# jhollowed/PyTEMDiags

Measured on AMD Instinct MI355X. Metric: grid-points/sec through full TEM pipeline (ncol*nlev*nt), higher is better.
Workload: dtype f64; 1 GPU; ne120 (777602 cols) x 72 lev x 30 snapshots per GPU, L=50, 1-degree zonal grid (M=180), ten GM16 Table-A1 outputs; ncol=777602, nlev=72, nt=30, sweeps=latitude-class, single sweep, mirror_paired_sweeps=True

## Files before the change

### include/temx.h

```cpp
#ifndef TEMX_H
#define TEMX_H

#include <stdint.h>

#ifdef __cplusplus
extern "C" {
#endif

typedef struct temx_plan temx_plan;

enum { TEMX_F64 = 0, TEMX_F32 = 1 };

enum {
  TEMX_OK = 0,
  TEMX_EINVAL = -1,
  TEMX_EHIP = -2,
  TEMX_ENOMEM = -3,
  TEMX_ERANK = -4,
  TEMX_ESTATE = -5,
  TEMX_EUNSUPPORTED = -6,
  TEMX_EINTERNAL = -7
};

enum {
  TEMX_DEFER_FINALIZE = 1,
  TEMX_NO_SYMMETRY = 2,
  TEMX_NO_CLASSES = 4,
  TEMX_NO_QR = 8,
  TEMX_LAT_TOL_F32 = 16
};

enum {
  TEMX_OPT_FORM = 1,
  TEMX_OPT_OS_MAP = 2,
  TEMX_OPT_OP_MAP = 3,
  TEMX_OPT_OS_SUBSAMPLE = 4,
  TEMX_OPT_TRACER_ONE_PASS = 5,
  TEMX_OPT_SINGLE_SWEEP_MIN_GROUPS = 6,
  TEMX_OPT_OS_CONTRACT = 7,
  TEMX_OPT_MISSING = 8,
  TEMX_OPT_MIN_COVERAGE = 9,
  TEMX_OPT_MISSING_WEIGHT = 10,
  TEMX_OPT_LAT_BINS = 12,
  TEMX_OPT_BIN_DEGREE = 13,
  TEMX_OPT_OS_SYNC = 11
};
enum {
  TEMX_FORM_AUTO = -1,
  TEMX_FORM_TWO_PASS = 0,
  TEMX_FORM_CLASS_SUMS = 1,
  TEMX_FORM_SINGLE_SWEEP = 2,
  TEMX_FORM_NO_SINGLE_SWEEP = 3,
  TEMX_FORM_MASKED = 4,
  TEMX_FORM_BINNED = 5
};

enum {
  TEMX_MAT_Y0 = 0,
  TEMX_MAT_Y0P = 1,
  TEMX_MAT_GRAM = 2,
  TEMX_MAT_GINV = 3,
  TEMX_MAT_Y0INV = 4,
  TEMX_MAT_GRAM2 = 5,
  TEMX_MAT_GX = 6,
  TEMX_MAT_GSUB = 7,
  TEMX_MAT_COVERAGE = 8
};

enum {
  TEMX_R_VTEM = 0, TEMX_R_OMEGATEM, TEMX_R_WTEM, TEMX_R_PSITEM, TEMX_R_EPFY, TEMX_R_EPFZ,
  TEMX_R_EPDIV, TEMX_R_UTENDEPFD, TEMX_R_UTENDVTEM, TEMX_R_UTENDWTEM, TEMX_NRESULTS
};

enum {
  TEMX_Z_UB = 0, TEMX_Z_VB, TEMX_Z_THETAB, TEMX_Z_WAPB, TEMX_Z_UPVPB, TEMX_Z_UPWAPPB,
  TEMX_Z_VPTPB, TEMX_Z_DUB_DP, TEMX_Z_DTHETAB_DP, TEMX_Z_UBCOSLAT, TEMX_Z_DUBCOSLAT_DLAT,
  TEMX_Z_PSI, TEMX_Z_PSICOSLAT, TEMX_Z_DPSICOSLAT_DLAT, TEMX_Z_DPSI_DP, TEMX_Z_INT_VBDP,
  TEMX_NZONAL
};

enum {
  TEMX_E_UP = 0, TEMX_E_VP, TEMX_E_THETAP, TEMX_E_WAPP, TEMX_E_UPVP, TEMX_E_UPWAPP, TEMX_E_VPTP,
  TEMX_NEDDY
};

int temx_version(void);
const char* temx_last_error(void);
int temx_device_count(void);

int temx_plan_create(temx_plan** out, int device, int64_t ncol, int L, int M,
                     const double* lat_deg_host, const double* lat_out_deg_host, int flags);

int temx_plan_finalize(temx_plan* plan, const double* G_host );

int temx_plan_refine(temx_plan* plan, const double* G2_host );

int temx_plan_set_weights(temx_plan* plan, const double* weights_host );

void temx_plan_destroy(temx_plan* plan);

int temx_plan_is_paired(const temx_plan* plan);
int temx_plan_sweep_mode(const temx_plan* plan);
int temx_plan_one_pass(const temx_plan* plan);
int temx_plan_single_sweep(const temx_plan* plan);

int temx_get_matrix(temx_plan* plan, int which, double* dst, void* stream);

int temx_plan_configure(temx_plan* plan, int option, int value);
int temx_plan_option(const temx_plan* plan, int option);

int temx_plan_set_os_matrices(temx_plan* plan, const double* Gx_host , const double* Gsub_host );


int temx_project(temx_plan* plan, const void* A, int dtype, int64_t D, double* B, void* stream);

int temx_zonal_mean(temx_plan* plan, const void* A, int dtype, int64_t D, double* out,
                    int native, void* stream);

int temx_zonal_mean_from_sums(temx_plan* plan, const double* B, int64_t D, double* out,
                              int native, void* stream);

int temx_plan_set_tem(temx_plan* plan, int nlev, int64_t nt, const double* p_pa_host, double p0);

int temx_tem_stage1(temx_plan* plan, const void* ua, const void* va, const void* ta,
                    const void* wap, int dtype, double* B4, void* stream);

int temx_tem_stage2(temx_plan* plan, const void* ua, const void* va, const void* ta,
                    const void* wap, int dtype, const double* B4, double* B3, void* stream);
// ... 76 lines not shown
```

### pytemdiags_amd/_lib.py

```python
from __future__ import annotations

import ctypes as C
import os

_HERE = os.path.dirname(os.path.abspath(__file__))
LIB_PATH = os.environ.get("TEMX_LIB") or os.path.join(_HERE, "libtemx.so")

ABI_VERSION = 402
F64, F32 = 0, 1
DEFER_FINALIZE = 1
NO_SYMMETRY = 2
NO_CLASSES = 4
NO_QR = 8
LAT_TOL_F32 = 16
MAT_Y0, MAT_Y0P, MAT_GRAM, MAT_GINV, MAT_Y0INV, MAT_GRAM2, MAT_GX, MAT_GSUB = 0, 1, 2, 3, 4, 5, 6, 7
MAT_COVERAGE = 8
OPT_FORM, OPT_OS_MAP, OPT_OP_MAP, OPT_OS_SUBSAMPLE, OPT_TRACER_ONE_PASS, OPT_SINGLE_SWEEP_MIN_GROUPS, OPT_OS_CONTRACT = 1, 2, 3, 4, 5, 6, 7
OPT_MISSING, OPT_MIN_COVERAGE, OPT_MISSING_WEIGHT = 8, 9, 10
OPT_OS_SYNC = 11
OPT_LAT_BINS, OPT_BIN_DEGREE = 12, 13
LAT_BINS_ALLOWED = (128, 256, 512, 1024, 2048)
LAT_BINS_DEFAULT = 512
MISSING_MODES = {"raise": 0, "mask": 1}
FORM_AUTO, FORM_TWO_PASS, FORM_CLASS_SUMS, FORM_SINGLE_SWEEP, FORM_NO_SINGLE_SWEEP = -1, 0, 1, 2, 3
FORM_MASKED = 4
FORM_BINNED = 5
FORM_NAMES = {FORM_TWO_PASS: "two-pass", FORM_CLASS_SUMS: "class-sums", FORM_SINGLE_SWEEP: "single-sweep",
              FORM_MASKED: "masked", FORM_BINNED: "binned"}
FORMS = {"auto": FORM_AUTO, "two-pass": FORM_TWO_PASS, "class-sums": FORM_CLASS_SUMS,
         "single-sweep": FORM_SINGLE_SWEEP, "no-single-sweep": FORM_NO_SINGLE_SWEEP}

RESULT_NAMES = ("vtem", "omegatem", "wtem", "psitem", "epfy", "epfz", "epdiv",
                "utendepfd", "utendvtem", "utendwtem")
ZONAL_NAMES = ("ub", "vb", "thetab", "wapb", "upvpb", "upwappb", "vptpb", "dub_dp", "dthetab_dp",
               "ubcoslat", "dubcoslat_dlat", "psi", "psicoslat", "dpsicoslat_dlat", "dpsi_dp",
               "int_vbdp")
EDDY_NAMES = ("up", "vp", "thetap", "wapp", "upvp", "upwapp", "vptp")
TRACER_RESULT_NAMES = ("etfy", "etfz", "etdiv", "qtendetfd", "qtendvtem", "qtendwtem")
TRACER_ZONAL_NAMES = ("qb", "qpvpb", "qpwappb", "dqb_dp", "qbcoslat", "dqbcoslat_dlat")
TRACER_EDDY_NAMES = ("qp", "qpvp", "qpwapp")

ERRORS = {0: "TEMX_OK", -1: "TEMX_EINVAL", -2: "TEMX_EHIP", -3: "TEMX_ENOMEM", -4: "TEMX_ERANK",
          -5: "TEMX_ESTATE", -6: "TEMX_EUNSUPPORTED", -7: "TEMX_EINTERNAL"}

_vp, _i, _i64, _dp, _u64 = C.c_void_p, C.c_int, C.c_int64, C.POINTER(C.c_double), C.c_uint64
SIGNATURES = [
    ("temx_version", _i, []),
    ("temx_last_error", C.c_char_p, []),
    ("temx_device_count", _i, []),
    ("temx_plan_create", _i, [C.POINTER(_vp), _i, _i64, _i, _i, _dp, _dp, _i]),
    ("temx_plan_finalize", _i, [_vp, _dp]),
    ("temx_plan_refine", _i, [_vp, _dp]),
    ("temx_plan_set_weights", _i, [_vp, _dp]),
    ("temx_plan_destroy", None, [_vp]),
    ("temx_plan_is_paired", _i, [_vp]),
    ("temx_plan_sweep_mode", _i, [_vp]),
    ("temx_plan_one_pass", _i, [_vp]),
    ("temx_plan_single_sweep", _i, [_vp]),
    ("temx_get_matrix", _i, [_vp, _i, _vp, _vp]),
    ("temx_plan_configure", _i, [_vp, _i, _i]),
    ("temx_plan_option", _i, [_vp, _i]),
    ("temx_plan_set_os_matrices", _i, [_vp, _dp, _dp]),
    ("temx_project", _i, [_vp, _vp, _i, _i64, _vp, _vp]),
    ("temx_zonal_mean", _i, [_vp, _vp, _i, _i64, _vp, _i, _vp]),
    ("temx_zonal_mean_from_sums", _i, [_vp, _vp, _i64, _vp, _i, _vp]),
    ("temx_plan_set_tem", _i, [_vp, _i, _i64, _dp, C.c_double]),
    ("temx_tem_stage1", _i, [_vp, _vp, _vp, _vp, _vp, _i, _vp, _vp]),
    ("temx_tem_stage2", _i, [_vp, _vp, _vp, _vp, _vp, _i, _vp, _vp, _vp]),
    ("temx_tem_stage2_from_sums", _i, [_vp, _vp, _vp, _vp]),
    ("temx_tem_stage3", _i, [_vp, _vp, _vp, _vp, _vp]),
    ("temx_tem_run", _i, [_vp, _vp, _vp, _vp, _vp, _i, _vp, _vp, _vp]),
    ("temx_tem_os_prepass", _i, [_vp, _vp, _vp, _vp, _vp, _i, _vp, _vp]),
    ("temx_tem_os_sweep", _i, [_vp, _vp, _vp, _vp, _vp, _i, _vp, _i, _vp, _vp]),
    ("temx_tem_os_tail", _i, [_vp, _vp, _i64, _i64, _vp, _vp, _vp]),
    ("temx_tracers_os_prepass", _i, [_vp, _i, C.POINTER(_vp), _vp, _vp, _i, _vp, _vp]),
    ("temx_tracers_os_sweep", _i, [_vp, _i, C.POINTER(_vp), _vp, _vp, _i, _vp, _i, _vp, _vp]),
    ("temx_tracers_os_tail", _i, [_vp, _i, _vp, C.POINTER(_vp), C.POINTER(_vp), _vp]),
    ("temx_tracers_run", _i, [_vp, _i, C.POINTER(_vp), _vp, _vp, _i, C.POINTER(_vp), C.POINTER(_vp), _vp]),
    ("temx_tem_tail_from_sums", _i, [_vp, _vp, _vp, _i64, _i64, _vp, _vp, _vp]),
    ("temx_time_slices", _i, [_vp, _vp, _i64, _i, _vp, _vp]),
    ("temx_tem_eddy", _i, [_vp, _vp, _vp, _vp, _vp, _i, C.POINTER(_vp), _vp]),
    ("temx_tem_eddy_rows", _i, [_vp, _vp, _vp, _vp, _vp, _i, _i64, _i64, C.POINTER(_vp), _vp]),
    ("temx_tracer_stage1", _i, [_vp, _vp, _i, _vp, _vp]),
    ("temx_tracer_stage2", _i, [_vp, _vp, _vp, _vp, _i, _vp, _vp, _vp]),
    ("temx_tracer_stage3", _i, [_vp, _vp, _vp, _vp, _vp]),
    ("temx_tracer_stage1_sums", _i, [_vp, _vp, _vp, _vp, _i, _vp, _vp]),
    ("temx_tracer_stage2_from_sums", _i, [_vp, _vp, _vp, _vp]),
    ("temx_tracer_run", _i, [_vp, _vp, _vp, _vp, _i, _vp, _vp, _vp]),
    ("temx_tem_tracer_stage1", _i, [_vp, _vp, _vp, _vp, _vp, _vp, _i, _vp, _vp, _vp]),
    ("temx_tem_tracer_run", _i, [_vp, _vp, _vp, _vp, _vp, _vp, _i, _vp, _vp, _vp, _vp, _vp]),
    ("temx_tracer_eddy", _i, [_vp, _vp, _vp, _vp, _i, C.POINTER(_vp), _vp]),
    ("temx_status", _i, [_vp, C.POINTER(_i), _vp]),
    ("temx_synth_fields", _i, [_i, _i64, _i, _i64, _i64, _vp, _vp, _vp, _i, _u64, _vp, _vp, _vp, _vp, _vp]),
    ("temx_mfma_f64_peak", _i, [_i, _i, _dp]),
    ("temx_kernel_timing", _i, [_vp, _i]),
    ("temx_kernel_timing_read", _i, [_vp, _i, _dp, C.POINTER(_i)]),
    ("temx_selftest_exception", _i, [_i]),
]


class TemxError(RuntimeError):
    def __init__(self, code, msg):
        super().__init__("%s (%d): %s" % (ERRORS.get(code, "TEMX_E?"), code, msg))
# ... 63 lines not shown
```

### pytemdiags_amd/csrc/kernels.hpp

```cpp
#pragma once
#include <hip/hip_runtime.h>
#include <stdint.h>

#include <type_traits>

#define TEMX_MFMA4(a, b, c) __builtin_amdgcn_mfma_f64_4x4x4f64((a), (b), (c), 0, 0, 0)

namespace temx {

template <int NF>
struct FieldPtrs {
  const void* p[NF];
};

struct EddyOut {
  double* p[7];
};

template <int KMAX>
__device__ __forceinline__ void basis_row(double xv, int K, const double* __restrict__ norm,
                                          const double* __restrict__ T, double* q) {
  double pm1 = 1.0, pc = xv;
  for (int l = 0; l < K; ++l) {
    double P;
// ... 163 lines not shown
          load_x(c0 + 1, std::integral_constant<int, (PD > 1 ? 1 : 0)>{}, ti, std::false_type{});
      }
      if (PD > 2 && c0 + 2 < c1) {
#pragma unroll
        for (int ti = 0; ti < 4; ++ti)
          load_x(c0 + 2, std::integral_constant<int, (PD > 2 ? 2 : 0)>{}, ti, std::false_type{});
      }
    }
  }
  const int cfast = (c1 < nfull ? c1 : nfull) - (2 * PD - 1);
  int chunk = c0;
  for (; chunk < cfast; chunk += PD) do_group(chunk, std::true_type{});
  for (; chunk < c1; chunk += PD) do_group(chunk, std::false_type{});

  if (dvalid) {
#pragma unroll
    for (int f = 0; f < NFW; ++f)
#pragma unroll
      for (int t = 0; t < TB; ++t) {
        const int l = t * 4 + g;
        if (l < K) partial[(((int64_t)split * NF + f0 + f) * K + l) * D + d] = acc[f][t];
      }
  }
}

struct SliceMap {
  int64_t D = 0;
  int nt = 1, W = 1;
  int64_t chunk = 0;
  int64_t row0 = 0;
};
__device__ __forceinline__ int64_t slice_index(const SliceMap& m, int64_t idx) {
  if (m.D == 0) return idx;
  const int64_t row = idx / m.D, d = idx - row * m.D;
  const int lev = (int)(d / m.nt), t = (int)(d - (int64_t)lev * m.nt);
  const int base = m.nt / m.W, extra = m.nt - base * m.W, tb = extra * (base + 1);
  int w, tl, ntw;
  if (t < tb) { w = t / (base + 1); tl = t - w * (base + 1); ntw = base + 1; }
  else { const int u = t - tb; w = extra + u / base; tl = u - (w - extra) * base; ntw = base; }
  const int nlev = (int)(m.D / m.nt);
  return (int64_t)w * m.chunk + ((m.row0 + row) * nlev + lev) * ntw + tl;
}

__global__ void __launch_bounds__(256)
reduce_partials_kernel(const double* __restrict__ partial, int nsplit, int64_t stride, int64_t n,
                       const double* __restrict__ addend, double* __restrict__ B, int* __restrict__ flag,
                       SliceMap map) {
  __shared__ double sh[16][17];
  const int e = threadIdx.x & 15, sl = threadIdx.x >> 4;
  const int64_t idx = (int64_t)blockIdx.x * 16 + e;
  double s = 0.0;
  if (idx < n)
    for (int sp = sl; sp < nsplit; sp += 16) s += partial[(int64_t)sp * stride + idx];
  sh[sl][e] = s;
  __syncthreads();
  if (sl == 0 && idx < n) {
    double t = 0.0;
#pragma unroll
    for (int j = 0; j < 16; ++j) t += sh[j][e];
    if (addend != nullptr) t += addend[idx];
    B[slice_index(map, idx)] = t;
    if (!(fabs(t) <= 1.79769313486231570815e308)) atomicOr(flag, 1);
  }
}

template <int NS>
__global__ void __launch_bounds__(256)
reduce_partials_flat_kernel(const double* __restrict__ partial, int nsplit, int64_t stride, int64_t n,
                            const double* __restrict__ addend, double* __restrict__ B, int* __restrict__ flag,
                            SliceMap map) {
  const int64_t idx = (int64_t)blockIdx.x * 256 + threadIdx.x;
  if (idx >= n) return;
  double v[NS];
#pragma unroll
  for (int sp = 0; sp < NS; ++sp) v[sp] = partial[(int64_t)(sp < nsplit ? sp : 0) * stride + idx];
  double t = 0.0;
#pragma unroll
  for (int sp = 0; sp < NS; ++sp) t += sp < nsplit ? v[sp] : 0.0;
  if (addend != nullptr) t += addend[idx];
  B[slice_index(map, idx)] = t;
  if (!(fabs(t) <= 1.79769313486231570815e308)) atomicOr(flag, 1);
}

__global__ void __launch_bounds__(256)
reduce_rows_kernel(const double* __restrict__ partial, int nsplit, int64_t stride, int nf, int rows_in, int rows,
                   int64_t D, double* __restrict__ out, int* __restrict__ flag) {
  const int64_t idx = (int64_t)blockIdx.x * 256 + threadIdx.x;
  const int64_t per = (int64_t)rows * D;
  if (idx >= per * nf) return;
  const int64_t f = idx / per, rem = idx - f * per;
  const double* src = partial + f * rows_in * D + rem;
  double t = 0.0;
  for (int sp = 0; sp < nsplit; ++sp) t += src[(int64_t)sp * stride];
  out[idx] = t;
  if (!(fabs(t) <= 1.79769313486231570815e308)) atomicOr(flag, 1);
}
__global__ void __launch_bounds__(256)
reduce_rows_wide_kernel(const double* __restrict__ partial, int nsplit, int64_t stride, int nf, int rows_in, int rows,
                        int64_t D, double* __restrict__ out, int* __restrict__ flag) {
  __shared__ double sh[16][17];
  const int e = threadIdx.x & 15, sl = threadIdx.x >> 4;
  const int64_t idx = (int64_t)blockIdx.x * 16 + e;
  const int64_t per = (int64_t)rows * D;
  const bool ok = idx < per * nf;
  double s = 0.0;
  if (ok) {
    const int64_t f = idx / per, rem = idx - f * per;
    const double* src = partial + f * rows_in * D + rem;
    for (int sp = sl; sp < nsplit; sp += 16) s += src[(int64_t)sp * stride];
  }
  sh[sl][e] = s;
  __syncthreads();
  if (sl == 0 && ok) {
    double t = 0.0;
#pragma unroll
    for (int j = 0; j < 16; ++j) t += sh[j][e];
    out[idx] = t;
    if (!(fabs(t) <= 1.79769313486231570815e308)) atomicOr(flag, 1);
  }
}

__global__ void __launch_bounds__(1024)
solve_kernel(const double* __restrict__ B, int K, int K4, int M, int64_t D,
             const double* __restrict__ Ginv, const double* __restrict__ Y0p,
             double* __restrict__ C, double* __restrict__ Xb) {
  extern __shared__ double slds[];
  double* sb = slds;
  double* scf = slds + (size_t)K4 * 17;
  const int f = blockIdx.y;
  const int64_t d0 = (int64_t)blockIdx.x * 16;
  const int tid = threadIdx.x;
  const int mper = (M + gridDim.z - 1) / gridDim.z;
  const int m0 = blockIdx.z * mper;
  const int m1 = m0 + mper < M ? m0 + mper : M;
  for (int idx = tid; idx < K * 16; idx += 1024) {
    const int k = idx >> 4, dd = idx & 15;
    const int64_t d = d0 + dd;
    sb[k * 17 + dd] = d < D ? B[((int64_t)f * K + k) * D + d] : 0.0;
  }
  __syncthreads();
  for (int idx = tid; idx < K4 * 16; idx += 1024) {
    const int k = idx >> 4, dd = idx & 15;
    const int64_t d = d0 + dd;
    double v = 0.0;
    if (k < K) {
      const double* gr = Ginv + (int64_t)k * K;
      double v0 = 0.0, v1 = 0.0, v2 = 0.0, v3 = 0.0;
      int kk = 0;
      for (; kk + 4 <= K; kk += 4) {
        v0 += gr[kk] * sb[kk * 17 + dd];
        v1 += gr[kk + 1] * sb[(kk + 1) * 17 + dd];
        v2 += gr[kk + 2] * sb[(kk + 2) * 17 + dd];
        v3 += gr[kk + 3] * sb[(kk + 3) * 17 + dd];
      }
      for (; kk < K; ++kk) v0 += gr[kk] * sb[kk * 17 + dd];
      v = (v0 + v1) + (v2 + v3);
    }
    scf[k * 17 + dd] = v;
    if (C != nullptr && blockIdx.z == 0 && d < D) C[((int64_t)f * K4 + k) * D + d] = v;
  }
  __syncthreads();
  if (Xb != nullptr) {
    for (int idx = tid; idx < (m1 - m0) * 16; idx += 1024) {
      const int m = m0 + (idx >> 4), dd = idx & 15;
      const int64_t d = d0 + dd;
      if (d >= D) continue;
      const double* yr = Y0p + (int64_t)m * K;
      double v0 = 0.0, v1 = 0.0, v2 = 0.0, v3 = 0.0;
      int kk = 0;
      for (; kk + 4 <= K; kk += 4) {
        v0 += yr[kk] * scf[kk * 17 + dd];
        v1 += yr[kk + 1] * scf[(kk + 1) * 17 + dd];
        v2 += yr[kk + 2] * scf[(kk + 2) * 17 + dd];
        v3 += yr[kk + 3] * scf[(kk + 3) * 17 + dd];
      }
      for (; kk < K; ++kk) v0 += yr[kk] * scf[kk * 17 + dd];
      Xb[((int64_t)f * M + m) * D + d] = (v0 + v1) + (v2 + v3);
    }
  }
}

constexpr int SOLVE_MB = 16;

template <int TB>
__global__ void __launch_bounds__(256)
solve_mfma_kernel(const double* __restrict__ B, int K, int M, int64_t D, const double* __restrict__ gblk,
                  const double* __restrict__ ypblk, double* __restrict__ C, double* __restrict__ Xb,
                  int mbs ) {
  extern __shared__ double slds[];
  double* sg = slds;
  double* sy = slds + TB * TB * 16;
  const int f = blockIdx.y;
  const int tid = threadIdx.x, lane = tid & 63, wave = tid >> 6;
  const int g = lane >> 4, c = lane & 15;
  const int64_t d = ((int64_t)blockIdx.x * 4 + wave) * 16 + c;
  const bool dvalid = d < D;
  const int64_t dcl = dvalid ? d : D - 1;
  const int mb0 = blockIdx.z * mbs;
  const int nmb_all = (M + 3) >> 2;
  const int nmb = Xb != nullptr ? (nmb_all - mb0 < mbs ? nmb_all - mb0 : mbs) : 0;

  double breg[TB];
#pragma unroll
  for (int t = 0; t < TB; ++t) {
    const int row = 4 * t + g;
    const int rc = row < K ? row : K - 1;
    const double v = B[((int64_t)f * K + rc) * D + dcl];
    breg[t] = row < K ? v : 0.0;
  }
  {
    constexpr int JG = (TB * TB * 16 + 255) / 256, JY = (SOLVE_MB * TB * 16 + 255) / 256;
    double tg[JG], ty[JY];
    const double* yp = ypblk + (int64_t)mb0 * TB * 16;
    const int ny = nmb * TB * 16;
#pragma unroll
    for (int j = 0; j < JG; ++j) tg[j] = gblk[tid + 256 * j < TB * TB * 16 ? tid + 256 * j : 0];
#pragma unroll
    for (int j = 0; j < JY; ++j) ty[j] = yp[tid + 256 * j < ny ? tid + 256 * j : 0];
#pragma unroll
    for (int j = 0; j < JG; ++j)
      if (tid + 256 * j < TB * TB * 16) sg[tid + 256 * j] = tg[j];
#pragma unroll
    for (int j = 0; j < JY; ++j)
      if (tid + 256 * j < ny) sy[tid + 256 * j] = ty[j];
  }
  __syncthreads();

  const uint32_t yoff = (uint32_t)(g * 4 + (lane & 3));
  double creg[TB];
#pragma unroll
  for (int r = 0; r < TB; ++r) creg[r] = 0.0;
#pragma unroll
  for (int t = 0; t < TB; ++t)
#pragma unroll
    for (int r = 0; r < TB; ++r) creg[r] = TEMX_MFMA4(sg[(r * TB + t) * 16 + yoff], breg[t], creg[r]);
  if (C != nullptr && blockIdx.z == 0 && dvalid) {
#pragma unroll
    for (int r = 0; r < TB; ++r) C[((int64_t)f * (4 * TB) + 4 * r + g) * D + d] = creg[r];
  }
  for (int mb = 0; mb < nmb; mb += 4) {
    double acc[4] = {0.0, 0.0, 0.0, 0.0};
#pragma unroll
    for (int t = 0; t < TB; ++t)
#pragma unroll
      for (int j = 0; j < 4; ++j) {
        const int mbj = mb + j < nmb ? mb + j : nmb - 1;
        acc[j] = TEMX_MFMA4(sy[(mbj * TB + t) * 16 + yoff], creg[t], acc[j]);
      }
#pragma unroll
    for (int j = 0; j < 4; ++j) {
      const int m = 4 * (mb0 + mb + j) + g;
      if (mb + j < nmb && m < M && dvalid) Xb[((int64_t)f * M + m) * D + d] = acc[j];
    }
  }
}

constexpr int EDDY_GR = 2;

template <typename T, int TB, int MODE, int DPW, int KIND>
__global__ void __launch_bounds__(512, 2)
eddy_kernel(FieldPtrs<4> fp, int64_t N, int64_t D, int K, const double* __restrict__ yblk,
            int64_t nchunk, const double* __restrict__ colscale,
            const double* __restrict__ C, double* __restrict__ partial, int nsplit, int ndt,
            EddyOut eo) {
  extern __shared__ double lds[];
  constexpr int GR = EDDY_GR;
  constexpr int YE = GR * TB * 16;
  constexpr int YJ = (YE + 63) / 64;
  constexpr int NP = 8 / DPW;
  constexpr bool TRACER = KIND == 1 || KIND == 3;
  constexpr int NFR = TRACER ? 3 : 4;
  constexpr int NPR = TRACER ? 2 : 3;
  int split, dq;
  if (!wg_work((ndt + DPW - 1) / DPW, nsplit, split, dq)) return;
  const int wave = uniform_wave(), lane = threadIdx.x & 63;
  const int w4 = wave % DPW, part = wave / DPW;
  const int c = lane & 15, g = lane >> 4;
  const int dt = dq * DPW + w4;
  const bool active = dt < ndt;
  const int64_t d = (int64_t)dt * 16 + c;
  const bool dvalid = active && d < D;
  const int64_t dcl = d < D ? d : D - 1;
// ... 568 lines not shown
```

### pytemdiags_amd/csrc/kernels_op2.hpp

```cpp
#pragma once
#include "kernels_op.hpp"

namespace temx {

template <int NA, int NB>
struct OpwSlot {
  double sd[2][NA][64];
  double y[NB * 16];
};

template <int TBS, int NA>
__device__ __forceinline__ void opw_round(const OpwSlot<NA, 2 * TBS>* slots, int par, int t0, int nbw,
                                          uint32_t yoff, int lane, double (&acc)[NA][(TBS + 1) / 2]) {
  asm volatile("s_waitcnt lgkmcnt(0)\n\ts_barrier" ::: "memory");
#pragma unroll
  for (int j = 0; j < 4; ++j) {
    double b[NA];
#pragma unroll
    for (int f = 0; f < NA; ++f) b[f] = slots[j].sd[par][f][lane];
#pragma unroll
    for (int tl = 0; tl < (TBS + 1) / 2; ++tl)
      if (tl < nbw) {
        const double ya = slots[j].y[(t0 + tl) * 16 + yoff];
#pragma unroll
// ... 498 lines not shown
      for (int k = 0; k < NP; ++k) q[k] = qN[k] = 0.0;
      cnt = cntN = 0.0;
    }
  };

  if (b0 < b1) {
    load_ys(grp);
    rn = crow[(int64_t)b0 * 4 + g];
    static_for<PD - 1>([&](auto kc) __attribute__((always_inline)) {
      constexpr int k = decltype(kc)::value;
      const int4 r0 = rn;
      rn = crow[(int64_t)(b0 + k + 1) * 4 + g];
      if (k == 0 || b0 + k < b1) issue(kc, r0);
    });
    constexpr int UNR = DEFER != 0 ? (PD % 4 == 0 ? PD : PD % 2 == 0 ? 2 * PD : 4 * PD) : PD;
    static_assert(UNR % PD == 0 && (DEFER == 0 || UNR % NCH == 0), "unrolled loop covers whole rings and whole chunk rounds");
    for (int b = b0; b < b1; b += UNR)
      static_for<UNR>([&](auto kc) __attribute__((always_inline)) {
        constexpr int k = decltype(kc)::value;
        if (k == 0 || b + k < b1) step(kc, b + k);
      });
  }
  if constexpr (DEFER != 0) {
    if (left > 0) {
      const int first = (b1 - b0) & (NCH - 1);
      static_for<NCH>([&](auto cc) __attribute__((always_inline)) {
        if (((decltype(cc)::value - first) & (NCH - 1)) < left) pending_chunk(cc);
      });
    }
  }
  if (dvalid) {
#pragma unroll
    for (int f = 0; f < NFX; ++f)
#pragma unroll
      for (int t = 0; t < NBX; ++t) {
        const int l = symx_harm<TBX>(t, g);
        if (l < (pp != nullptr ? KX : K4)) px[(((int64_t)split * NFX + f) * KX + l) * D + d] = ax[f][t];
      }
#pragma unroll
    for (int k = 0; k < NP; ++k)
#pragma unroll
      for (int t = 0; t < 2 * TBS; ++t) {
        const int l = sym_harm<TBS>(t, g);
        if (pp != nullptr && l < K) pp[(((int64_t)split * NP + k) * K + l) * D + d] = apl[(k * 2 * TBS + t) * 64];
      }
  }
}

#ifndef TEMX_ROWLOAD_MOD
#define TEMX_ROWLOAD_MOD "nt"
#endif
template <typename T> struct RowLoad;
template <> struct RowLoad<double> {
  static __device__ __forceinline__ void ld(double& dst, uint32_t voff, uint64_t sbase) {
    asm volatile("global_load_dwordx2 %0, %1, %2 " TEMX_ROWLOAD_MOD : "=v"(dst) : "v"(voff), "s"(sbase) : "memory");
  }
};
template <> struct RowLoad<float> {
  static __device__ __forceinline__ void ld(float& dst, uint32_t voff, uint64_t sbase) {
    asm volatile("global_load_dword %0, %1, %2 " TEMX_ROWLOAD_MOD : "=v"(dst) : "v"(voff), "s"(sbase) : "memory");
  }
};
__device__ __forceinline__ double temx_rcp_count(double n) {
  double r = __builtin_amdgcn_rcp(n);
  return __builtin_fma(__builtin_fma(-n, r, 1.0), r, r);
}
template <int N, typename T>
__device__ __forceinline__ void row_wait(T& a, T& b, T& c, T& d) {
  asm volatile("s_waitcnt vmcnt(%4)" : "+v"(a), "+v"(b), "+v"(c), "+v"(d) : "n"(N) : "memory");
}
template <int N, typename T>
__device__ __forceinline__ void row_wait(T& a, T& b, T& c) {
  asm volatile("s_waitcnt vmcnt(%3)" : "+v"(a), "+v"(b), "+v"(c) : "n"(N) : "memory");
}
template <typename T>
__device__ __forceinline__ void row_touch(T& a) {
  asm volatile("" : "+v"(a)::"memory");
}

constexpr int HANDOFF_LOOKS = 1 << 22;
__device__ __forceinline__ uint32_t handoff_look(const uint32_t* ctr) {
  return __hip_atomic_load(ctr, __ATOMIC_RELAXED, __HIP_MEMORY_SCOPE_WORKGROUP);
}
template <typename T, int TBS, int TBX, int NBR, int PD, int KIND = 0, int SYNC = 0>
__global__ void __launch_bounds__(256, 1)
sweep_osr_kernel(FieldPtrs<4> fp, int64_t D, int K, int KX, const double* __restrict__ ycx,
                 const int4* __restrict__ crow, const int2* __restrict__ csplit,
                 const double* __restrict__ colscale, const double* __restrict__ rho, int K4,
                 double* __restrict__ px, double* __restrict__ pp, int nsplit, int ndt, int* __restrict__ hstat) {
  using KD = OsKind<KIND>;
  constexpr int NF = KD::NF, NFX = KD::NFX, NP = KD::NP;
  constexpr int NBX = 2 * TBX;
  constexpr int YE = NBX * 16;
  constexpr int YJ = (YE + 255) / 256;
  constexpr int MB = CLS_MB;
  constexpr int NCH = 4;
  constexpr int NV = 2 * (NF + NP);
  constexpr int NPR = KD::NPR, NPL = NP - NPR;
  static_assert(NBR <= TBS && TBS <= TBX, "reference degree <= L <= 2L");
  static_assert(YJ <= 2, "Y quarter per thread");
  static_assert((PD - 1) * CLS_MB * KD::NF + (CLS_MB - 1) * KD::NF + 2 <= 63, "the ring is counted in vmcnt (6 bits)");
  extern __shared__ double lds[];
  int split, dq;
  if (!wg_work((ndt + 3) / 4, nsplit, split, dq)) return;
  const int tid = threadIdx.x;
  const int wave = uniform_wave(), lane = tid & 63;
  const int c = lane & 15, g = lane >> 4;
  const int64_t colr = (int64_t)dq * 64 + lane < D ? (int64_t)dq * 64 + lane : D - 1;
  const uint32_t colb32 = (uint32_t)colr * (uint32_t)sizeof(T);
  const int dt = dq * 4 + wave;
  const int64_t d = (int64_t)dt * 16 + c;
  const bool dvalid = dt < ndt && d < D;
  const int64_t dcl = dvalid ? d : D - 1;
  const int b0 = __builtin_amdgcn_readfirstlane(csplit[split].x);
  const int b1 = __builtin_amdgcn_readfirstlane(csplit[split + 1].x);
  int grp = __builtin_amdgcn_readfirstlane(csplit[split].y);
  const uint32_t aoff_p = (uint32_t)(g * 4 + (lane & 3));
  const uint32_t aoff_r = (uint32_t)((lane & 3) * 4 + g);
  double* ybase = lds;
  double* cn = lds + 2 * YE;
  double* cb = lds + 2 * YE + 16 + wave * (NF * 2 * NBR * 64) + lane;
  double* apl = lds + 2 * YE + 16 + 4 * (NF * 2 * NBR * 64) + wave * (NPL * 2 * TBS * 64) + lane;
  double* ex = lds + 2 * YE + 16 + 4 * (NF * 2 * NBR * 64) + 4 * (NPL * 2 * TBS * 64);
  double* exw = ex + wave * 64 + lane;
  const double* exr = ex + g * 64 + wave * 16 + c;
  uint32_t* hctr = reinterpret_cast<uint32_t*>(ex + NV * 256);
  const double sth = (KD::TF >= 0 && colscale != nullptr) ? colscale[colr] : 1.0;
  if constexpr (SYNC != 0) {
    if (tid < 2) hctr[tid] = 0u;
    __syncthreads();
  }
#pragma unroll
  for (int i = 0; i < NPL * 2 * TBS; ++i) apl[i * 64] = 0.0;
  double apr[NPR > 0 ? NPR : 1][2 * TBS];
#pragma unroll
  for (int k = 0; k < (NPR > 0 ? NPR : 1); ++k)
#pragma unroll
    for (int t = 0; t < 2 * TBS; ++t) apr[k][t] = 0.0;
#pragma unroll
  for (int f = 0; f < NF; ++f)
#pragma unroll
    for (int tb = 0; tb < 2 * NBR; ++tb) {
      const int l = tb < NBR ? 2 * (4 * tb + g) : 2 * (4 * (tb - NBR) + g) + 1;
      const double v = rho[((int64_t)f * K4 + (l < K ? l : K - 1)) * D + dcl];
      cb[(f * 2 * NBR + tb) * 64] = l < K ? v : 0.0;
    }
  uint64_t fbase[NF];
#pragma unroll
  for (int f = 0; f < NF; ++f) fbase[f] = reinterpret_cast<uint64_t>(fp.p[f]);
  { double sth_ready = sth; asm volatile("" : "+v"(sth_ready)); }

  double ax[NFX][NBX];
#pragma unroll
  for (int f = 0; f < NFX; ++f)
#pragma unroll
    for (int t = 0; t < NBX; ++t) ax[f][t] = 0.0;
  double s[NF], q[NP], x0[NF], cnt = 0.0;
  double sN[NF], qN[NP], x0N[NF], cntN = 0.0;
#pragma unroll
  for (int f = 0; f < NF; ++f) s[f] = x0[f] = sN[f] = x0N[f] = 0.0;
#pragma unroll
  for (int k = 0; k < NP; ++k) q[k] = qN[k] = 0.0;
  bool north_open = false, prev_south = false;
  const uint32_t rowbytes = (uint32_t)D * (uint32_t)sizeof(T);

  T xb[PD][MB][NF];
  int er[PD][MB];
  double ys[YJ];
  const uint32_t yoff32[2] = {(uint32_t)(tid < YE ? tid : 0) * 8u, (uint32_t)(tid + 256 < YE ? tid + 256 : 0) * 8u};
  auto load_ys = [&](int gi) __attribute__((always_inline)) {
#pragma unroll
    for (int j = 0; j < YJ; ++j) RowLoad<double>::ld(ys[j], yoff32[j], reinterpret_cast<uint64_t>(ycx) + (uint64_t)gi * (YE * 8));
  };
  auto issue = [&](auto pc, const int4 rv) __attribute__((always_inline)) {
    constexpr int P = decltype(pc)::value;
    er[P][0] = rv.x; er[P][1] = rv.y; er[P][2] = rv.z; er[P][3] = rv.w;
#pragma unroll
    for (int j = 0; j < MB; ++j) {
      const uint64_t off = (uint64_t)(uint32_t)(er[P][j] & CLS_ROWMASK) * rowbytes;
#pragma unroll
      for (int f = 0; f < NF; ++f) RowLoad<T>::ld(xb[P][j][f], colb32, fbase[f] + off);
    }
  };
  double dS[NFX][2], dP[NP][2];
  const double* yprev = ybase;
  int ycur = 0;
  int left = 0;
#pragma unroll
  for (int f = 0; f < NFX; ++f) dS[f][0] = dS[f][1] = 0.0;
#pragma unroll
  for (int k = 0; k < NP; ++k) dP[k][0] = dP[k][1] = 0.0;
  auto pending_chunk = [&](auto cc) __attribute__((always_inline)) {
    constexpr int C = decltype(cc)::value;
#pragma unroll
    for (int t = C * NBX / NCH; t < (C + 1) * NBX / NCH; ++t) {
      const double ya = yprev[t * 16 + aoff_p];
#pragma unroll
      for (int f = 0; f < NFX; ++f) ax[f][t] = TEMX_MFMA4(ya, dS[f][t < TBX ? 0 : 1], ax[f][t]);
      const int tp = t < TBX ? t : t - TBX;
      if (tp < TBS) {
        const int ta = t < TBX ? tp : TBS + tp;
#pragma unroll
        for (int k = 0; k < NPR; ++k) apr[k][ta] = TEMX_MFMA4(ya, dP[k][t < TBX ? 0 : 1], apr[k][ta]);
        if constexpr (NPL > 0) {
          double v[NPL > 0 ? NPL : 1];
#pragma unroll
          for (int k = 0; k < NPL; ++k) v[k] = apl[(k * 2 * TBS + ta) * 64];
#pragma unroll
          for (int k = 0; k < NPL; ++k) v[k] = TEMX_MFMA4(ya, dP[NPR + k][t < TBX ? 0 : 1], v[k]);
#pragma unroll
          for (int k = 0; k < NPL; ++k) apl[(k * 2 * TBS + ta) * 64] = v[k];
        }
      }
    }
  };
  auto park_north = [&]() __attribute__((always_inline)) {
#pragma unroll
    for (int f = 0; f < NF; ++f) { sN[f] = s[f]; x0N[f] = x0[f]; s[f] = 0.0; }
#pragma unroll
    for (int k = 0; k < NP; ++k) { qN[k] = q[k]; q[k] = 0.0; }
    cntN = cnt;
    cnt = 0.0;
  };
  auto tile_role = [&](const double* yw) __attribute__((always_inline)) {
    double m2[2][NF], c2[2][NP];
#pragma unroll
    for (int f = 0; f < NF; ++f) {
      m2[0][f] = exr[f * 256];
      m2[1][f] = exr[(NF + NP + f) * 256];
    }
#pragma unroll
    for (int k = 0; k < NP; ++k) {
      c2[0][k] = exr[(NF + k) * 256];
      c2[1][k] = exr[(2 * NF + NP + k) * 256];
    }
    const double nN = cn[g], nS = cn[4 + g];
    double E[NF], O[NF];
#pragma unroll
    for (int f = 0; f < NF; ++f) E[f] = O[f] = 0.0;
#pragma unroll
    for (int tb = 0; tb < ((TEMX_OS_SKIP & 2) ? 0 : 2 * NBR); ++tb) {
      const int blk = tb < NBR ? tb : TBX + (tb - NBR);
      const double ya = yw[blk * 16 + aoff_r];
#pragma unroll
      for (int f = 0; f < NF; ++f) {
        if (tb < NBR)
          E[f] = TEMX_MFMA4(ya, cb[(f * 2 * NBR + tb) * 64], E[f]);
        else
          O[f] = TEMX_MFMA4(ya, cb[(f * 2 * NBR + tb) * 64], O[f]);
      }
    }
    if constexpr (SYNC != 0) {
      asm volatile("s_waitcnt lgkmcnt(0)" ::: "memory");
      if (lane == 0) __hip_atomic_fetch_add(&hctr[1], 1u, __ATOMIC_RELAXED, __HIP_MEMORY_SCOPE_WORKGROUP);
    }
#pragma unroll
    for (int f = 0; f < NF; ++f) {
      m2[0][f] -= E[f] + O[f];
      m2[1][f] -= E[f] - O[f];
    }
#pragma unroll
    for (int f = 0; f < NFX; ++f) {
      const double SNf = nN * m2[0][f], SSf = nS * m2[1][f];
      dS[f][0] = SNf + SSf;
      dS[f][1] = SNf - SSf;
    }
#pragma unroll
    for (int k = 0; k < NP; ++k) {
      const double PNk = c2[0][k] + nN * m2[0][KD::pa(k)] * m2[0][KD::pb(k)];
      const double PSk = c2[1][k] + nS * m2[1][KD::pa(k)] * m2[1][KD::pb(k)];
      dP[k][0] = PNk + PSk;
      dP[k][1] = PNk - PSk;
    }
    yprev = yw;
    left = NCH;
  };
  uint32_t hgen = 0;
  bool hpend = false;
  int hfail = 0;
  const double* ypend = ybase;
  auto handoff_wait = [&](const uint32_t* ctr, uint32_t seen, uint32_t need, int code) __attribute__((always_inline)) {
    seen = (uint32_t)__builtin_amdgcn_readfirstlane((int)seen);
    if (seen >= need || hfail != 0) return;
#pragma unroll 1
    for (int n = 0; n < HANDOFF_LOOKS; ++n) {
      __builtin_amdgcn_s_sleep(1);
      seen = (uint32_t)__builtin_amdgcn_readfirstlane((int)handoff_look(ctr));
      if (seen >= need) return;
    }
    hfail = code;
  };
  int4 rn;
  auto step = [&](auto posc, int b) __attribute__((always_inline)) {
    constexpr int POS = decltype(posc)::value % NCH;
    constexpr int P = decltype(posc)::value % PD;
    uint32_t seen = 0;
    if constexpr (SYNC != 0) {
      if (hpend) seen = handoff_look(&hctr[0]);
    }
    {
      const int4 r1 = rn;
      rn = crow[(int64_t)(b + PD) * 4 + wave];
      issue(std::integral_constant<int, (P + PD - 1) % PD>{}, r1);
    }
    if constexpr (SYNC != 0) {
      if (hpend) {
        if (left > 0)
          static_for<NCH>([&](auto cc) __attribute__((always_inline)) {
            if (((decltype(cc)::value - POS) & (NCH - 1)) < left) pending_chunk(cc);
          });
        handoff_wait(&hctr[0], seen, 4u * hgen, 1);
        tile_role(ypend);
        hpend = false;
      }
    }
    if (left > 0) {
      if (!(TEMX_OS_SKIP & 1)) pending_chunk(std::integral_constant<int, POS>{});
      --left;
    }
    static_assert(NF == 4 || NF == 3, "row_wait has forms for 3 and 4 fields");
    static_for<MB>([&](auto jc) __attribute__((always_inline)) {
      constexpr int j = decltype(jc)::value;
      constexpr int NW = (PD - 1) * MB * NF + (MB - 1 - j) * NF;
      if constexpr (NF == 4) row_wait<NW>(xb[P][j][0], xb[P][j][1], xb[P][j][2], xb[P][j][3]);
      else row_wait<NW>(xb[P][j][0], xb[P][j][1], xb[P][j][2]);
    });
#pragma unroll
    for (int j = 0; j < YJ; ++j) row_touch(ys[j]);
    const int fl = er[P][0] >> 27;
    const bool south = (fl & (CLS_SOUTH << 1)) != 0;
    if ((fl & (CLS_FIRST << 1)) || (south && !prev_south)) {
      if (south && north_open) park_north();
      north_open = !south;
#pragma unroll
      for (int f = 0; f < NF; ++f) x0[f] = (double)xb[P][0][f];
    }
    prev_south = south;
#pragma unroll
    for (int j = 0; j < ((TEMX_OS_SKIP & 4) ? 0 : MB); ++j) {
      const double w = er[P][j] < 0 ? 0.0 : 1.0;
      double dx[NF];
#pragma unroll
      for (int f = 0; f < NF; ++f) dx[f] = (double)xb[P][j][f] - x0[f];
#pragma unroll
      for (int f = 0; f < NF; ++f) s[f] += w * dx[f];
#pragma unroll
      for (int k = 0; k < NP; ++k) q[k] += (w * dx[KD::pa(k)]) * dx[KD::pb(k)];
      cnt += w;
    }
    if (fl & (CLS_LAST << 1)) {
      prev_south = false;
      if (north_open) park_north();
      north_open = false;
      uint32_t seen_done = 0;
      if constexpr (SYNC == 0) {
        if (left > 0)
          static_for<NCH>([&](auto cc) __attribute__((always_inline)) {
            if (((decltype(cc)::value - POS - 1) & (NCH - 1)) < left) pending_chunk(cc);
          });
      } else {
        seen_done = handoff_look(&hctr[1]);
      }
      const double rnN = cntN > 0.0 ? temx_rcp_count(cntN) : 0.0, rnS = cnt > 0.0 ? temx_rcp_count(cnt) : 0.0;
      double val[NV];
#pragma unroll
      for (int f = 0; f < NF; ++f) {
        const double sc = f == KD::TF ? sth : 1.0;
        val[f] = (sN[f] * rnN + x0N[f]) * sc;
        val[NF + NP + f] = (s[f] * rnS + x0[f]) * sc;
      }
#pragma unroll
      for (int k = 0; k < NP; ++k) {
        const double sc = k == KD::TP ? sth : 1.0;
        val[NF + k] = (qN[k] - sN[KD::pa(k)] * sN[KD::pb(k)] * rnN) * sc;
        val[2 * NF + NP + k] = (q[k] - s[KD::pa(k)] * s[KD::pb(k)] * rnS) * sc;
      }
      if constexpr (SYNC == 0) {
        if (!(TEMX_OS_SKIP & 8)) asm volatile("s_waitcnt lgkmcnt(0)\n\ts_barrier" ::: "memory");
      } else {
        handoff_wait(&hctr[1], seen_done, 4u * hgen, 2);
      }
      ycur ^= 1;
      double* yw = ybase + ycur * YE;
#pragma unroll
      for (int v = 0; v < NV; ++v) exw[v * 256] = val[v];
      if (lane == 0) {
        cn[wave] = cntN;
        cn[4 + wave] = cnt;
      }
#pragma unroll
      for (int j = 0; j < YJ; ++j)
        if (tid + 256 * j < YE) yw[tid + 256 * j] = ys[j];
      if constexpr (SYNC == 0) {
        if (!(TEMX_OS_SKIP & 8)) asm volatile("s_waitcnt lgkmcnt(0)\n\ts_barrier" ::: "memory");
      } else {
        asm volatile("s_waitcnt lgkmcnt(0)" ::: "memory");
        if (lane == 0) __hip_atomic_fetch_add(&hctr[0], 1u, __ATOMIC_RELAXED, __HIP_MEMORY_SCOPE_WORKGROUP);
        ++hgen;
        hpend = true;
        ypend = yw;
      }
      ++grp;
      load_ys(grp);
      if constexpr (SYNC == 0) tile_role(yw);
#pragma unroll
      for (int f = 0; f < NF; ++f) s[f] = sN[f] = 0.0;
#pragma unroll
      for (int k = 0; k < NP; ++k) q[k] = qN[k] = 0.0;
      cnt = cntN = 0.0;
    }
  };

  if (b0 < b1) {
    load_ys(grp);
    rn = crow[(int64_t)b0 * 4 + wave];
    static_for<PD - 1>([&](auto kc) __attribute__((always_inline)) {
      constexpr int k = decltype(kc)::value;
      const int4 r0 = rn;
      rn = crow[(int64_t)(b0 + k + 1) * 4 + wave];
      issue(kc, r0);
    });
    constexpr int UNR = PD % 4 == 0 ? PD : PD % 2 == 0 ? 2 * PD : 4 * PD;
    for (int b = b0; b < b1; b += UNR)
      static_for<UNR>([&](auto kc) __attribute__((always_inline)) {
        constexpr int k = decltype(kc)::value;
        if (k == 0 || b + k < b1) step(kc, b + k);
      });
    asm volatile("s_waitcnt vmcnt(0)" ::: "memory");
  }
  if constexpr (SYNC != 0) {
    if (hpend) {
      if (left > 0) {
        const int first = (b1 - b0) & (NCH - 1);
        static_for<NCH>([&](auto cc) __attribute__((always_inline)) {
          if (((decltype(cc)::value - first) & (NCH - 1)) < left) pending_chunk(cc);
        });
      }
      handoff_wait(&hctr[0], handoff_look(&hctr[0]), 4u * hgen, 1);
      tile_role(ypend);
    }
    if (hfail != 0 && lane == 0) atomicOr(hstat, hfail);
  }
  if (left > 0) {
    const int first = (b1 - b0) & (NCH - 1);
    static_for<NCH>([&](auto cc) __attribute__((always_inline)) {
      if (((decltype(cc)::value - first) & (NCH - 1)) < left) pending_chunk(cc);
    });
  }
  if (dvalid) {
#pragma unroll
    for (int f = 0; f < NFX; ++f)
#pragma unroll
      for (int t = 0; t < NBX; ++t) {
        const int l = symx_harm<TBX>(t, g);
        if (l < (pp != nullptr ? KX : K4)) px[(((int64_t)split * NFX + f) * KX + l) * D + d] = ax[f][t];
      }
#pragma unroll
    for (int k = 0; k < NP; ++k)
#pragma unroll
      for (int t = 0; t < 2 * TBS; ++t) {
        const int l = sym_harm<TBS>(t, g);
        if (pp != nullptr && l < K) pp[(((int64_t)split * NP + k) * K + l) * D + d] = k < NPR ? apr[k < NPR ? k : 0][t] : apl[((k < NPR ? 0 : k - NPR) * 2 * TBS + t) * 64];
      }
  }
}

#ifndef TEMX_OS2_STAGGER
#define TEMX_OS2_STAGGER 0
#endif
#ifndef TEMX_OS2_ACC32
#define TEMX_OS2_ACC32 1
#endif
template <typename T, int TBS, int TBX, int NBR, int PD, int KIND = 0>
__global__ void __launch_bounds__(512, 1)
sweep_os2_kernel(FieldPtrs<4> fp, int64_t D, int K, int KX, const double* __restrict__ ycx,
                 const int4* __restrict__ crowN, const int4* __restrict__ crowS,
                 const int* __restrict__ gfirstN, const int* __restrict__ gfirstS, const int2* __restrict__ csplit,
                 const double* __restrict__ colscale, const double* __restrict__ rho, int K4,
                 double* __restrict__ px, double* __restrict__ pp, int nsplit, int ndt) {
  using KD = OsKind<KIND>;
  constexpr int NF = KD::NF, NFX = KD::NFX, NP = KD::NP;
  constexpr int NBX = 2 * TBX;
  constexpr int YE = NBX * 16;
  constexpr int MB = CLS_MB;
  constexpr int NCH = 2;
  constexpr int NV = NF + NP;
  constexpr int NPR = KD::NPR, NPL = NP - NPR;
  static_assert(NBR <= TBS && TBS <= TBX, "reference degree <= L <= 2L");
  static_assert(YE <= 512, "one Y element per thread");
  static_assert((PD - 1) * MB * NF + (MB - 1) * NF + 1 <= 63, "the ring is counted in vmcnt (6 bits)");
  extern __shared__ double lds[];
  int split, dq;
  if (!wg_work((ndt + 3) / 4, nsplit, split, dq)) return;
  const int tid = threadIdx.x;
  const int wave = uniform_wave(), lane = tid & 63;
  const int c = lane & 15, g = lane >> 4;
  const int side = wave >> 2;
  const int64_t colr = (int64_t)dq * 64 + lane < D ? (int64_t)dq * 64 + lane : D - 1;
  const uint32_t colb32 = (uint32_t)colr * (uint32_t)sizeof(T);
  const int tl = wave & 3, par = wave >> 2;
  const int dt = dq * 4 + tl;
  const int64_t d = (int64_t)dt * 16 + c;
  const bool dvalid = dt < ndt && d < D;
  const int64_t dcl = dvalid ? d : D - 1;
  const int4* __restrict__ crow = side ? crowS : crowN;
  const int* __restrict__ gfirst = side ? gfirstS : gfirstN;
  int grp = __builtin_amdgcn_readfirstlane(csplit[split].y);
  const int grp1 = __builtin_amdgcn_readfirstlane(csplit[split + 1].y);
  const int b0 = __builtin_amdgcn_readfirstlane(gfirst[grp]);
  const int b1 = __builtin_amdgcn_readfirstlane(gfirst[grp1]);
  const uint32_t aoff_p = (uint32_t)(g * 4 + (lane & 3));
  const uint32_t aoff_r = (uint32_t)((lane & 3) * 4 + g);
  double* ybase = lds;
  double* cn = lds + 2 * YE;
  double* cb = lds + 2 * YE + 16 + tl * (NF * 2 * NBR * 64) + lane;
  double* apl = lds + 2 * YE + 16 + 4 * (NF * 2 * NBR * 64) + wave * (NPL * TBS * 64) + lane;
  double* ex = lds + 2 * YE + 16 + 4 * (NF * 2 * NBR * 64) + 8 * (NPL * TBS * 64);
  double* exw = ex + wave * 64 + lane;
  const double* exr = ex + g * 64 + tl * 16 + c;
  const double sth = (KD::TF >= 0 && colscale != nullptr) ? colscale[colr] : 1.0;
#pragma unroll
  for (int i = 0; i < NPL * TBS; ++i) apl[i * 64] = 0.0;
  double apr[NPR > 0 ? NPR : 1][TBS];
#pragma unroll
  for (int k = 0; k < (NPR > 0 ? NPR : 1); ++k)
#pragma unroll
    for (int t = 0; t < TBS; ++t) apr[k][t] = 0.0;
  if (par == 0) {
#pragma unroll
    for (int f = 0; f < NF; ++f)
// ... 395 lines not shown
#pragma unroll
      for (int f = 0; f < NST; ++f) {
        ex[f][wave][lane] = sN[f] + sS[f];
        ex[NA + f][wave][lane] = sN[f] - sS[f];
      }
#pragma unroll
      for (int k = 0; k < NQ; ++k) {
        ex[NST + k][wave][lane] = qN[k] + qS[k];
        ex[NA + NST + k][wave][lane] = qN[k] - qS[k];
      }
      if (tid < YE) ybuf[ycur][tid] = ys;
      asm volatile("s_waitcnt lgkmcnt(0)\n\ts_barrier" ::: "memory");
      ++grp;
      load_ys(grp);
#pragma unroll
      for (int f = 0; f < NA; ++f) {
        pS[f] = ex[f][g][wave * 16 + c];
        pD[f] = ex[NA + f][g][wave * 16 + c];
      }
      yprev = ybuf[ycur];
      left = NCH;
#pragma unroll
      for (int f = 0; f < NST; ++f) sN[f] = 0.0;
#pragma unroll
      for (int k = 0; k < NQ; ++k) qN[k] = 0.0;
    }
  };

  if (b0 < b1) {
    load_ys(grp);
    rn = crow[(int64_t)b0 * 4 + wave];
    static_for<PD - 1>([&](auto kc) __attribute__((always_inline)) {
      constexpr int k = decltype(kc)::value;
      const int4 r0 = rn;
      rn = crow[(int64_t)(b0 + k + 1) * 4 + wave];
      issue(kc, r0);
    });
    constexpr int UNR = PD % 4 == 0 ? PD : PD % 2 == 0 ? 2 * PD : 4 * PD;
    for (int b = b0; b < b1; b += UNR)
      static_for<UNR>([&](auto kc) __attribute__((always_inline)) {
        constexpr int k = decltype(kc)::value;
        if (k == 0 || b + k < b1) step(kc, b + k);
      });
    asm volatile("s_waitcnt vmcnt(0)" ::: "memory");
  }
  if (left > 0) {
    const int first = (b1 - b0) & (NCH - 1);
    static_for<NCH>([&](auto cc) __attribute__((always_inline)) {
      if (((decltype(cc)::value - first) & (NCH - 1)) < left) pending_chunk(cc);
    });
  }
  if (dvalid) {
#pragma unroll
    for (int f = 0; f < NA; ++f)
#pragma unroll
      for (int t = 0; t < NB; ++t) {
        const int l = sym_harm<TBS>(t, g);
        if (l < K) partial[(((int64_t)split * NA + f) * K + l) * D + d] = acc[f][t];
      }
  }
}

__global__ void __launch_bounds__(256)
os_ref_solve_kernel(const double* __restrict__ As, int KX , int KR, int64_t D,
                    const double* __restrict__ Gsinv, double* __restrict__ rho) {
  __shared__ double sg[16 * 16];
  const int f = blockIdx.y;
  for (int i = threadIdx.x; i < KR * KR; i += blockDim.x) sg[i] = Gsinv[i];
  __syncthreads();
  const int64_t d = blockIdx.x * (int64_t)(blockDim.x / 16) + (threadIdx.x & 15);
  const int l = threadIdx.x >> 4;
  if (d >= D || l >= KR) return;
  const double* a = As + (int64_t)f * KX * D + d;
  double v0 = 0.0, v1 = 0.0;
  int m = 0;
  for (; m + 2 <= KR; m += 2) {
    v0 += sg[l * KR + m] * a[(int64_t)m * D];
    v1 += sg[l * KR + m + 1] * a[(int64_t)(m + 1) * D];
  }
  if (m < KR) v0 += sg[l * KR + m] * a[(int64_t)m * D];
  rho[((int64_t)f * KR + l) * D + d] = v0 + v1;
}

constexpr int OSC = 4;
constexpr int OSR = 256 / OSC;

__device__ __forceinline__ void os_stage(double* dst, const double* __restrict__ src, int n, int tid) {
  for (int i = tid; i < n; i += 256) dst[i] = src[i];
}

__host__ __device__ inline size_t os_contract_lds(int K, int KX, int NQ) {
  const size_t big = (size_t)NQ * KX > (size_t)2 * K * K ? (size_t)NQ * KX : (size_t)2 * K * K;
  return ((size_t)4 * KX + 8 * K + 8 * NQ + 3 * KX + 3 * K) * OSC + big;
}

struct OsFields {
  const double* A[4];
  const double* rho[4];
};

template <int KIND>
__global__ void __launch_bounds__(256)
os_contract_kernel(OsFields in, const double* __restrict__ Pp,
                   int K, int KX, int KR, int NQ, int64_t D, const double* __restrict__ Tm,
                   const double* __restrict__ G2inv, const double* __restrict__ G, const double* __restrict__ Gx,
                   const double* __restrict__ Yq, const double* __restrict__ wq2, double* __restrict__ B4,
                   double* __restrict__ B3, int64_t Drho, int nts, int nt, int t0) {
  using KD = OsKind<KIND>;
  constexpr int NF = KD::NF, NP = KD::NP, NOUT = KIND == 0 ? 4 : 1;
  static_assert(OSC == 4, "a thread owns one output row for the four columns of the workgroup");
  extern __shared__ double sm[];
  const int KK = K * K;
  double* sA = sm;
  double* sAl = sA + 4 * KX * OSC;
  double* sW = sAl + 4 * K * OSC;
  double* sAt = sW + 4 * K * OSC;
  double* sAb = sAt + 4 * NQ * OSC;
  double* sC = sAb + 4 * NQ * OSC;
  double* sF = sC + 3 * KX * OSC;
  double* big = sF + 3 * K * OSC;
  const int tid = threadIdx.x;
  const int64_t d0 = (int64_t)blockIdx.x * OSC;
  auto dot4 = [&](const double* mrow, int mstride, const double* v, int n, double (&acc)[OSC]) __attribute__((always_inline)) {
#pragma unroll 8
    for (int k = 0; k < n; ++k) {
      const double m = mrow[(size_t)k * mstride];
      const double4 x = *reinterpret_cast<const double4*>(v + k * OSC);
      acc[0] += m * x.x; acc[1] += m * x.y; acc[2] += m * x.z; acc[3] += m * x.w;
    }
  };
  auto put4 = [&](double* dst, const double (&a)[OSC]) __attribute__((always_inline)) {
    *reinterpret_cast<double4*>(dst) = make_double4(a[0], a[1], a[2], a[3]);
  };
  for (int i = tid; i < NF * KX * OSC; i += 256) {
    const int row = i / OSC, c = i % OSC;
    const int64_t d = d0 + c < D ? d0 + c : D - 1;
    sA[i] = in.A[row / KX][(int64_t)(row % KX) * D + d];
  }
  os_stage(big, Tm, KK, tid);
  os_stage(big + KK, G2inv, KK, tid);
  __syncthreads();
  const double* sT = big;
  const double* sG2 = big + KK;
  for (int i = tid; i < NF * K; i += 256) {
    const int f = i / K, j = i % K;
    double a[OSC] = {0.0, 0.0, 0.0, 0.0};
    dot4(sT + j, K, sA + (size_t)f * KX * OSC, j + 1, a);
    put4(sW + (size_t)i * OSC, a);
  }
  __syncthreads();
  for (int i = tid; i < NF * K; i += 256) {
    const int f = i / K, j = i % K;
    double a[OSC] = {0.0, 0.0, 0.0, 0.0};
    dot4(sG2 + j * K, 1, sW + (size_t)f * K * OSC, K, a);
    put4(sAl + (size_t)i * OSC, a);
  }
  __syncthreads();
  for (int i = tid; i < NF * K; i += 256) {
    const int f = i / K, l = i % K;
    double a[OSC] = {0.0, 0.0, 0.0, 0.0};
    dot4(sT + l * K + l, 1, sAl + ((size_t)f * K + l) * OSC, K - l, a);
    put4(sW + (size_t)i * OSC, a);
  }
  __syncthreads();
  for (int i = tid; i < K * KR; i += 256) big[KK + i] = G[(i / KR) * K + (i % KR)];
  for (int i = tid; i < NOUT * KR * OSC; i += 256) {
// ... 84 lines not shown
```

### pytemdiags_amd/csrc/temx.hip

```cpp
#include "../../include/temx.h"
#include "../../include/temx_vert.h"
#include "../../include/temx_layout.h"
#include "../../include/temx_ingest.h"
#include "../../include/temx_clim.h"
#include "../../include/temx_mtracer.h"
#include "../../include/temx_nclim.h"
#include "../../include/temx_gclim.h"
#include "../include/temx_mgclim.h"
#include "../include/temx_wave.h"

#include <hip/hip_runtime.h>

#include <algorithm>
#include <cmath>
#include <cstdarg>
#include <cstdio>
#include <cstdlib>
#include <cstring>
#include <map>
#include <mutex>
#include <new>
#include <stdexcept>
#include <string>
#include <thread>
// ... 61 lines not shown
  size_t bytes = 0;
  int ensure(size_t need) {
    if (need <= bytes) return TEMX_OK;
    if (p) (void)hipFree(p);
    p = nullptr;
    bytes = 0;
    hipError_t e = hipMalloc(&p, need);
    if (e != hipSuccess) return fail(TEMX_ENOMEM, "hipMalloc(%zu) failed: %s", need, hipGetErrorString(e));
    bytes = need;
    return TEMX_OK;
  }
  void release() {
    if (p) (void)hipFree(p);
    p = nullptr;
    bytes = 0;
  }
  double* d() const { return static_cast<double*>(p); }
};

struct TimedLaunch {
  hipEvent_t a, b;
};

struct temx_plan {
  int device = 0, num_cu = 256;
  int64_t N = 0, nchunk = 0;
  int L = 0, K = 0, TB = 0, K4 = 0, M = 0;
  int stride = 0, nslice = 1;
  bool large = false;
  DevBuf Bs, XB, P3;
  bool finalized = false;
  bool weighted = false;
  int rank = 0;
  DevBuf x, Y0, yblk, yblk_w, Y0p, G, Ginv, norm, flag;
  DevBuf gblk, ypblk;
  bool qbasis = false;
  bool g_checker = false;
  bool ext_G = false;
  bool os_need_global = false;
  DevBuf T, Qp, GinvA, G2, xo, xc;
  int64_t cls_npad = 0;
  const double* yproj_ptr() const { return yblk_w.p ? yblk_w.d() : yblk.d(); }
  std::vector<double> lat_out_deg;
  bool tem = false;
  int nlev = 0;
  int64_t nt = 0, D = 0;
  double p0 = 101325.0;
  DevBuf p, pg, lg, coslat, fcor, colscale;
  DevBuf B4, B3, C4, zb;
  DevBuf Bq, Bq2, Ct, tz;
  Split sp_proj1;
  bool sym = false;
  int TBS = 0;
  int64_t npair = 0, npg = 0, npg_alloc = 0;
  DevBuf rows, ysym;
  Split sp_sproj4, sp_sproj1, sp_seddy;
  Split sp_proj4, sp_eddy;
  bool cls = false;
  int64_t cgroups = 0, cbatches = 0, ncls = 0;
  int64_t cls_max_side = 0;
  std::vector<int> gbatch0;
  DevBuf crow, ycls;
  std::map<int, DevBuf> csplits;
  Split sp_cproj4, sp_cproj1, sp_ceddy, sp_cflux;
  bool os_built = false, os_on = false;
  bool os_valid = false;
  DevBuf Axq, rho_t;
  int TBX = 0, KX = 0, KR = 0, NQ = 0;
  std::vector<double> h_xc, h_cnt;
  std::vector<int> h_crow;
  std::vector<int> sgbatch0;
  int64_t sgroups = 0, sbatches = 0;
  DevBuf ycx, ycx_s, crow_s, rho, rho0, gaunt , wq2, Gx, Gsinv, Ax , Axs ;
  std::vector<double> h_G_own;
  std::vector<double> h_Gx_own;
  std::vector<double> h_Gx, h_Gs;
  std::vector<double> h_T, h_Ginv, h_G, h_Yq;
  DevBuf oscblk, osAt, osAb, osAtq, osAbq, Bqp;
  OscMats osc{};
  bool osc_lds = false;
  int opt_os_contract = -1;
  bool os_barrier = false;
  int opt_os_sync = -1;
  int os_keep = 32;
  int64_t tD = 0, tnt = 0, tt0 = 0;
  int opt_form = -1, opt_os_map = -1, opt_op_map = -1, opt_tracer_one_pass = -1, opt_single_sweep_min_groups = -1;
  bool os_tile = false, op_tile = false;
  bool no_qr = false;
  DevBuf side_crow[2][2], side_gfirst[2][2];
  std::map<int, DevBuf> csplits_s;
  Split sp_os, sp_os_s;
  Split sp_copw;
  bool lcls = false, lone = false, xb_valid = false;
  DevBuf ycls_l, pbuf;
  int64_t ycls_lstride = 0;
  Split sp_lflux;
  bool onepass = false, op_valid = false;
  bool c4_valid = false;
  DevBuf csum, ccnt;
  DevBuf Pq;
  DevBuf csq, Pq2;
  bool tq_valid = false;
  DevBuf partial;
  DevBuf opB, opC;
  int opt_missing = 0, opt_min_cov = 500, opt_miss_w = 10;
  bool miss_built = false;
  bool miss_valid = false;
  int64_t miss_cov_D = -1;
  int NE = 0, NQM = 0;
  DevBuf eblk;
  DevBuf mtab;
  DevBuf mB, mC, mCcov, mcov, mZ;
  bool mt_valid = false;
  DevBuf mtB, mtB2, mtC, mtCcov, mtz;
  int opt_lat_bins = 0;
  int bin_J = 0, bin_KP = 0;
  int bin_built = 0;
  int bin_pass = 0;
  int64_t bin_nchunk = 0;
  std::vector<double> h_lat;
  DevBuf bin_a, bin_chunk, bin_c0, bin_rows, bin_s;
  DevBuf bin_T;
  DevBuf bin_cm, bin_z, bin_cy;
  bool timing = false;
  std::vector<TimedLaunch> timed[2];
};

static int upload(DevBuf& b, const void* src, size_t bytes) {
  int rc = b.ensure(bytes);
  if (rc) return rc;
  HIPCHK(hipMemcpy(b.p, src, bytes, hipMemcpyHostToDevice));
  return TEMX_OK;
}

__global__ void fill_zero_kernel(double2* __restrict__ p, int64_t n) {
  const double2 z = make_double2(0.0, 0.0);
  for (int64_t i = blockIdx.x * (int64_t)blockDim.x + threadIdx.x; i < n; i += (int64_t)gridDim.x * blockDim.x) p[i] = z;
}

static int alloc_write_stream(DevBuf& b, size_t need) {
  need = (need + 15) & ~(size_t)15;
  if (b.bytes >= need) return TEMX_OK;
  int tries = 4;
  if (const char* e = getenv("TEMX_PLACE_TRIES")) tries = std::max(1, std::min(8, atoi(e)));
  if (need < ((size_t)1 << 30)) tries = 1;
  b.release();
  std::vector<DevBuf> cand;
  std::vector<float> ms;
  hipEvent_t ea = nullptr, eb = nullptr;
  if (tries > 1 && (hipEventCreate(&ea) != hipSuccess || hipEventCreate(&eb) != hipSuccess)) tries = 1;
  int best = -1;
  float slowest = 0.f;
  for (int t = 0; t < tries; ++t) {
    size_t fr = 0, tot = 0;
    if (t > 0 && (hipMemGetInfo(&fr, &tot) != hipSuccess || need > fr / 2)) break;
    DevBuf c;
    if (c.ensure(need) != TEMX_OK) {
      if (t == 0) return TEMX_ENOMEM;
      break;
    }
    float best_ms = 1e30f;
    for (int rep = 0; rep < (tries > 1 ? 2 : 1); ++rep) {
      if (ea) (void)hipEventRecord(ea, nullptr);
      hipLaunchKernelGGL(fill_zero_kernel, dim3(2048), dim3(256), 0, nullptr, static_cast<double2*>(c.p), (int64_t)(need / 16));
      if (ea) {
        float m = 0.f;
// ... 75 lines not shown
  (void)hipEventCreate(&tl.b);
  (void)hipEventRecord(tl.a, st);
}
static void time_end(temx_plan* pl, int which, hipStream_t st, TimedLaunch& tl) {
  if (!pl->timing || tl.a == nullptr) return;
  (void)hipEventRecord(tl.b, st);
  pl->timed[which].push_back(tl);
}

struct ProjCfgC { static constexpr int NFW = 4, PD = 1, WPS = 2; };
struct ProjCfgE { static constexpr int NFW = 1, PD = 2, WPS = 3; };
struct ProjCfg1 { static constexpr int NFW = 1, PD = 2, WPS = 2; };

static int pick_dpw(int ndt, int maxdpw) {
  int best = maxdpw;
  double bw = 1e9;
  for (int d = maxdpw; d >= 1; d >>= 1) {
    const double w = (double)(((ndt + d - 1) / d) * d) / ndt;
    if (w < bw - 0.05) {
      bw = w;
      best = d;
    }
  }
  return best;
}
static int proj_dpw(int NF, int ndt) {
  if (NF == 1) return 4;
  return pick_dpw(ndt, 4) == 1 ? 1 : 4;
}
static int proj_wps(int NF, int dpw) {
  if (NF == 1) return ProjCfg1::WPS;
  return dpw == 1 ? ProjCfgE::WPS : ProjCfgC::WPS;
}

constexpr int SYM_PROJ_E_WPS = 3;
struct ProjCfg3 { static constexpr int NFW = 3, PD = 1, WPS = 2; };

template <int NF>
static int launch_project(temx_plan* pl, const FieldPtrs<NF>& fp, int dtype, int64_t D,
                          const double* colscale, int sfield, double* partial, const Split& sp,
                          hipStream_t st, int tb_off = 0, int Kloc = -1) {
  if (Kloc < 0) Kloc = pl->K;
  return by_dtype(dtype, [&](auto t) {
    using T = typename decltype(t)::type;
    auto go = [&](auto cfg) {
      using Cfg = decltype(cfg);
      return dispatch(TBValues{}, pl->TB, [&](auto tb) {
        return launch<project_kernel<T, NF, Cfg::NFW, decltype(tb)::value, Cfg::PD, Cfg::WPS>>(
            dim3(sp.grid), dim3(256), 0, st, fp, pl->N, D, Kloc, pl->yproj_ptr(), pl->stride, tb_off, pl->nchunk, colscale,
            sfield, partial, sp.nsplit, sp.ndt);
      });
    };
    if constexpr (NF == 1) return go(ProjCfg1{});
    else if constexpr (NF == 3) return go(ProjCfg3{});
    else return sp.dpw == 1 ? go(ProjCfgE{}) : go(ProjCfgC{});
  });
}

static int launch_reduce(temx_plan* pl, const double* partial, int nsplit, int64_t n, double* B,
                         hipStream_t st, int64_t stride = -1, const double* addend = nullptr,
                         const SliceMap& map = SliceMap(), int* flag = nullptr) {
  if (stride < 0) stride = n;
  if (flag == nullptr) flag = static_cast<int*>(pl->flag.p);
  if (nsplit <= 16 && n >= 32768) {
    const dim3 grid((unsigned)((n + 255) / 256));
    if (nsplit <= 2)
      hipLaunchKernelGGL(reduce_partials_flat_kernel<2>, grid, dim3(256), 0, st, partial, nsplit, stride, n, addend, B, flag, map);
    else if (nsplit <= 4)
      hipLaunchKernelGGL(reduce_partials_flat_kernel<4>, grid, dim3(256), 0, st, partial, nsplit, stride, n, addend, B, flag, map);
    else if (nsplit <= 8)
      hipLaunchKernelGGL(reduce_partials_flat_kernel<8>, grid, dim3(256), 0, st, partial, nsplit, stride, n, addend, B, flag, map);
    else
      hipLaunchKernelGGL(reduce_partials_flat_kernel<16>, grid, dim3(256), 0, st, partial, nsplit, stride, n, addend, B, flag, map);
    HIPCHK(hipGetLastError());
    return TEMX_OK;
  }
  const int64_t blocks = (n + 15) / 16;
  hipLaunchKernelGGL(reduce_partials_kernel, dim3((unsigned)blocks), dim3(256), 0, st, partial, nsplit, stride, n,
                     addend, B, flag, map);
  HIPCHK(hipGetLastError());
  return TEMX_OK;
}

static int launch_reduce_rows(temx_plan* pl, const double* partial, int nsplit, int64_t stride, int nf, int rows_in,
                              int rows, int64_t D, double* out, hipStream_t st) {
  const int64_t n = (int64_t)nf * rows * D;
  if (nsplit > 16)
    hipLaunchKernelGGL(reduce_rows_wide_kernel, dim3((unsigned)((n + 15) / 16)), dim3(256), 0, st, partial, nsplit, stride,
                       nf, rows_in, rows, D, out, static_cast<int*>(pl->flag.p));
  else
    hipLaunchKernelGGL(reduce_rows_kernel, dim3((unsigned)((n + 255) / 256)), dim3(256), 0, st, partial, nsplit, stride,
                       nf, rows_in, rows, D, out, static_cast<int*>(pl->flag.p));
  HIPCHK(hipGetLastError());
  return TEMX_OK;
}

static int launch_solve(temx_plan* pl, const double* B, int NF, int64_t D, double* C, double* Xb,
                        hipStream_t st) {
  if (pl->K <= 64) {
    const int nmb = (pl->M + 3) / 4;
    const int gx = (int)(((D + 15) / 16 + 3) / 4);
    int mbs = SOLVE_MB;
    while (mbs > 4 && (int64_t)gx * NF * ((nmb + mbs - 1) / mbs) < pl->num_cu / 2) mbs -= 4;
    dim3 grid((unsigned)gx, NF, Xb ? (nmb + mbs - 1) / mbs : 1);
    return dispatch(TBValues{}, pl->TB, [&](auto tb) {
      constexpr int TBv = decltype(tb)::value;
      const size_t slds = ((size_t)TBv * TBv + (size_t)SOLVE_MB * TBv) * 16 * sizeof(double);
      return launch_lds<solve_mfma_kernel<TBv>>(pl->device, grid, dim3(256), slds, st, B, pl->K, pl->M, D, pl->gblk.d(),
                                                pl->ypblk.d(), C, Xb, mbs);
    });
  }
  const int ms = Xb ? (pl->M + 63) / 64 : 1;
  dim3 grid((unsigned)((D + 15) / 16), NF, ms);
  const size_t slds = (size_t)2 * pl->K4 * 17 * sizeof(double);
  return launch_lds<solve_kernel, 160 * 1024>(pl->device, grid, dim3(1024), slds, st, B, pl->K, pl->K4, pl->M, D,
      pl->Ginv.d(), pl->Qp.d(), C, Xb);
}

template <typename T, int MODE, int KIND>
static int launch_eddy_t(temx_plan* pl, const FieldPtrs<4>& fp, const double* C, double* partial,
                         const Split& sp, const EddyOut& eo, hipStream_t st) {
  constexpr int NFR = (KIND == 1 || KIND == 3) ? 3 : 4;
  return dispatch(DpwValues{}, sp.dpw, [&](auto dpw) {
    return dispatch(TBValues{}, pl->TB, [&](auto tb) {
      constexpr int DPW = decltype(dpw)::value, TBv = decltype(tb)::value;
      const size_t lds = ((size_t)DPW * NFR * TBv * 64 + 8 * EDDY_GR * TBv * 16) * sizeof(double);
      return launch_lds<eddy_kernel<T, TBv, MODE, DPW, KIND>>(pl->device, dim3(sp.grid), dim3(512), lds, st, fp, pl->N, pl->D,
                                                              pl->K, pl->yblk.d(), pl->nchunk, pl->colscale.d(), C, partial,
                                                              sp.nsplit, sp.ndt, eo);
    });
  });
}

static int launch_recon(temx_plan* pl, int64_t D, const double* C, double* out, hipStream_t st,
                        int64_t row0 = 0, int64_t nrows = -1) {
  if (nrows < 0) nrows = pl->N - row0;
  const int64_t nch = (nrows + 15) / 16;
  const double* yb0 = pl->yblk.d() + (row0 / 4) * pl->stride * 16;
  Split sp = choose_split(D, nch, 2 * pl->num_cu);
  dim3 grid(sp.grid), block(256);
  if (pl->large) {
    for (int sl = 0; sl < pl->nslice; ++sl)
      hipLaunchKernelGGL(recon_kernel<16>, grid, block, (size_t)4 * 16 * 64 * sizeof(double), st, nrows, D, yb0, pl->stride,
          16 * sl, nch, C + (int64_t)64 * sl * D, out, sl > 0 ? 1 : 0, sp.nsplit, sp.ndt);
    HIPCHK(hipGetLastError());
    return TEMX_OK;
  }
  return dispatch(TBValues{}, pl->TB, [&](auto tb) {
    constexpr int TBv = decltype(tb)::value;
    return launch<recon_kernel<TBv>>(grid, block, (size_t)4 * TBv * 64 * sizeof(double), st, nrows, D, yb0, pl->stride, 0,
        nch, C, out, 0, sp.nsplit, sp.ndt);
  });
}

template <int NF>
static int project_all(temx_plan* pl, const FieldPtrs<NF>& fp, int dtype, int64_t D, const double* colscale,
                       int sfield, const Split& sp, double* B, hipStream_t st) {
  int rc;
  if (!pl->large) {
    if ((rc = launch_project<NF>(pl, fp, dtype, D, colscale, sfield, pl->partial.d(), sp, st))) return rc;
    return launch_reduce(pl, pl->partial.d(), sp.nsplit, (int64_t)NF * pl->K * D, B, st);
  }
  if ((rc = pl->Bs.ensure((size_t)NF * 64 * D * 8))) return rc;
  for (int sl = 0; sl < pl->nslice; ++sl) {
    const int Ks = std::min(64, pl->K - 64 * sl);
    if ((rc = launch_project<NF>(pl, fp, dtype, D, colscale, sfield, pl->partial.d(), sp, st, 16 * sl, Ks))) return rc;
    if ((rc = launch_reduce(pl, pl->partial.d(), sp.nsplit, (int64_t)NF * Ks * D, pl->Bs.d(), st))) return rc;
    for (int f = 0; f < NF; ++f)
      HIPCHK(hipMemcpyAsync(B + ((int64_t)f * pl->K + 64 * sl) * D, pl->Bs.d() + (int64_t)f * Ks * D,
                            (size_t)Ks * D * 8, hipMemcpyDeviceToDevice, st));
  }
  return TEMX_OK;
}

static double sym_tol_deg(double dflt) {
  double tol = dflt;
  if (const char* e = getenv("TEMX_SYM_TOL_DEG")) {
    const double t = atof(e);
    if (t > 0.0 && t < 1e-3) tol = t;
  }
  return tol;
}

static int cached_cuts(std::map<int, DevBuf>& cache, const std::vector<int>& gbatch0, int64_t ngroups, int64_t nbatches,
                       int nsub, bool group_aligned, const int2** out) {
  const int key = group_aligned ? -nsub : nsub;
  auto it = cache.find(key);
  if (it == cache.end()) {
    DevBuf b;
    if (int rc = upload(b, work_cuts(gbatch0, ngroups, nbatches, nsub, group_aligned))) return rc;
    it = cache.emplace(key, b).first;
  }
  *out = static_cast<const int2*>(it->second.p);
  return TEMX_OK;
}
static int class_cuts_dev(temx_plan* pl, int nsub, const int2** out, bool group_aligned = false) {
  return cached_cuts(pl->csplits, pl->gbatch0, pl->cgroups, pl->cbatches, nsub, group_aligned, out);
}
static int os_cuts_dev(temx_plan* pl, bool sub, int nsub, const int2** out) {
// ... 301 lines not shown
    const QuadBasis qb = quadrature_basis(nq, KX);
    pl->h_Yq.assign(qb.Y.begin(), qb.Y.end());
    if ((rc = upload(pl->gaunt, pl->h_Yq))) return rc;
    if ((rc = upload(pl->wq2, std::vector<double>(qb.w2.begin(), qb.w2.end())))) return rc;
  }
  pl->h_Gx = extended_gram(pl->h_xc, pl->h_cnt, pl->ncls, K, KX, (int)std::max(1u, std::min(16u, std::thread::hardware_concurrency())));
  pl->h_Gx_own = pl->h_Gx;
  if ((rc = upload(pl->Gx, pl->h_Gx))) return rc;
  pl->os_built = true;
  return os_upload_blocks(pl);
}

static int os_upload_blocks(temx_plan* pl) {
  if (pl->h_T.empty() || pl->h_Ginv.empty() || pl->h_G.empty() || pl->h_Yq.empty() || pl->h_Gx.empty()) return TEMX_OK;
  const int K = pl->K, KX = pl->KX, KR = pl->KR, NQ = pl->NQ;
  const int NBK = pl->TB, NBX = 2 * pl->TBX;
  if (4 * NBK < K || 4 * NBX < KX || 4 * NBX < NQ) return fail(TEMX_EUNSUPPORTED, "single-sweep contraction: no instantiation for L = %d", pl->L);
  std::vector<double> blk;
  size_t off[9];
  const double* T = pl->h_T.data();
  const double* Yq = pl->h_Yq.data();
  off[0] = blk.size(); append_blocks16(blk, T, K, K, K, true, NBK, NBK);
  off[1] = blk.size(); append_blocks16(blk, pl->h_Ginv.data(), K, K, K, false, NBK, NBK);
  off[2] = blk.size(); append_blocks16(blk, T, K, K, K, false, NBK, NBK);
  off[3] = blk.size(); append_blocks16(blk, pl->h_G.data(), K, KR, K, false, NBK, 4);
  off[4] = blk.size(); append_blocks16(blk, Yq, NQ, K, KX, false, NBX, NBK);
  off[5] = blk.size(); append_blocks16(blk, Yq, NQ, KX, KX, false, NBX, NBX);
  off[6] = blk.size(); append_blocks16(blk, Yq, K, NQ, KX, true, NBK, NBX);
  off[7] = blk.size(); append_blocks16(blk, Yq, KX, NQ, KX, true, NBX, NBX);
  off[8] = blk.size(); append_blocks16(blk, pl->h_Gx.data(), K, KX, KX, false, NBK, NBX);
  HIPCHK(hipDeviceSynchronize());
  if (int rc = upload(pl->oscblk, blk.data(), blk.size() * 8)) return rc;
  const double* b = pl->oscblk.d();
  pl->osc = OscMats{b + off[0], b + off[1], b + off[2], b + off[3], b + off[4], b + off[5], b + off[6], b + off[7], b + off[8]};
  return TEMX_OK;
}

#ifndef TEMX_OS_DEFER
#define TEMX_OS_DEFER 1
#endif
template <typename T, int KIND>
static int launch_sweep_os_t(temx_plan* pl, const FieldPtrs<4>& fp, bool sub, const double* rho, double* partial,
                             const Split& sp, hipStream_t st) {
  using KD = OsKind<KIND>;
  const int2* cuts = nullptr;
  if (int rc = os_cuts_dev(pl, sub, sp.nsplit, &cuts)) return rc;
  dim3 grid(sp.grid), block(256);
  constexpr int NBR = 2;
  constexpr int PDv = sizeof(T) == 4 ? 4 : 2;
  constexpr int DF = TEMX_OS_DEFER;
  const bool tile_map = pl->os_tile;
  double* px = partial;
  double* pp = sub ? nullptr : partial + (int64_t)sp.nsplit * KD::NFX * pl->KX * pl->D;
  int rc = TEMX_OK;
  const bool listed = dispatch_strict(OsPairs{}, pl->TBS, pl->TBX, rc, [&](auto pair) {
    constexpr int TBSv = decltype(pair)::first, TBXv = decltype(pair)::second;
    if constexpr (KIND == 3) {
      if (tile_map) return fail(TEMX_EUNSUPPORTED, "two tracers per sweep: row-map sweeps only");
    }
    if constexpr (KIND != 3) if (tile_map) {
      const size_t lds = ((size_t)4 * (DF ? 2 : 1) * 2 * TBXv * 16 + (size_t)4 * KD::NF * 2 * NBR * 64 +
                          (size_t)4 * KD::NP * 2 * TBSv * 64) * 8;
      return launch_lds<sweep_os_kernel<T, TBSv, TBXv, NBR, PDv, KIND, DF>>(pl->device, grid, block, lds, st, fp, pl->D,
          pl->K, pl->KX, sub ? pl->ycx_s.d() : pl->ycx.d(), static_cast<const int4*>(sub ? pl->crow_s.p : pl->crow.p), cuts,
          pl->colscale.d(), rho, pl->KR, px, pp, sp.nsplit, sp.ndt);
    }
    if (sizeof(T) == 4) {
      if (pl->cls_max_side > 8 * TEMX_F32_SIDE_CAP)
        return fail(TEMX_EUNSUPPORTED, "single sweep of fp32 fields: a latitude class of this plan has %lld members on one "
                    "side, and the sweep sums a side in fp32; create the plan with TEMX_LAT_TOL_F32",
                    (long long)pl->cls_max_side);
      const size_t lds = ((size_t)2 * 2 * TBXv * 16 + 16 + (size_t)4 * KD::NF * 2 * NBR * 64 +
                          (size_t)8 * (KD::NP - KD::NPR) * TBSv * 64 + (size_t)(KD::NF + KD::NP) * 512) * 8;
      const int si = sub ? 1 : 0;
      return launch_lds<sweep_os2_kernel<float, TBSv, TBXv, NBR, 2, KIND>>(
          pl->device, grid, dim3(512), lds, st, fp, pl->D, pl->K, pl->KX, sub ? pl->ycx_s.d() : pl->ycx.d(),
          static_cast<const int4*>(pl->side_crow[si][0].p), static_cast<const int4*>(pl->side_crow[si][1].p),
          static_cast<const int*>(pl->side_gfirst[si][0].p), static_cast<const int*>(pl->side_gfirst[si][1].p),
          cuts, pl->colscale.d(), rho, pl->KR, px, pp, sp.nsplit, sp.ndt);
    }
    constexpr size_t lds = ((size_t)2 * 2 * TBXv * 16 + 16 + (size_t)4 * KD::NF * 2 * NBR * 64 +
                            (size_t)4 * (KD::NP - KD::NPR) * 2 * TBSv * 64 + (size_t)2 * (KD::NF + KD::NP) * 256 + 2) * 8;
    static_assert(lds <= 163840, "the single sweep's workgroup fits the LDS of a compute unit");
    auto go = [&](auto handoff) {
      return launch_lds<sweep_osr_kernel<double, TBSv, TBXv, NBR, 2, KIND, decltype(handoff)::value>>(pl->device, grid,
          block, lds, st, fp, pl->D, pl->K, pl->KX, sub ? pl->ycx_s.d() : pl->ycx.d(),
          static_cast<const int4*>(sub ? pl->crow_s.p : pl->crow.p), cuts, pl->colscale.d(), rho, pl->KR, px, pp, sp.nsplit,
          sp.ndt, static_cast<int*>(pl->flag.p) + 1);
    };
    return pl->os_barrier ? go(Int<0>{}) : go(Int<1>{});
  });
  return listed ? rc : fail(TEMX_EUNSUPPORTED, "single-sweep form: no instantiation for L = %d", pl->L);
}

template <int KIND>
static int launch_sweep_os(temx_plan* pl, const FieldPtrs<4>& fp, int dtype, bool sub, const double* rho, double* partial,
                           const Split& sp, hipStream_t st) {
  return dtype == TEMX_F64 ? launch_sweep_os_t<double, KIND>(pl, fp, sub, rho, partial, sp, st)
                           : launch_sweep_os_t<float, KIND>(pl, fp, sub, rho, partial, sp, st);
}

static bool os_supported(const temx_plan* pl) {
  if (!pl->cls || pl->large || pl->weighted || !pl->qbasis || pl->h_crow.empty()) return false;
  const int tbx = (pl->L + 1 + 3) / 4;
  return (pl->TBS == 7 && tbx <= 13) || (pl->TBS == 4 && tbx <= 8) || (pl->TBS == 2 && tbx <= 4);
}

static bool os_active(const temx_plan* pl, int dtype) {
  (void)dtype;
  return pl->os_on;
}

static void set_tail(temx_plan* pl, int64_t t0, int64_t nts) {
  if (pl->tt0 != t0 || pl->tnt != nts) pl->c4_valid = pl->os_valid = pl->op_valid = pl->tq_valid = pl->xb_valid = false;
  pl->tt0 = t0;
  pl->tnt = nts;
  pl->tD = (int64_t)pl->nlev * nts;
}
static inline bool tail_is_whole(const temx_plan* pl) { return pl->tt0 == 0 && pl->tnt == pl->nt; }

static int tem_stage3_impl(temx_plan* pl, const double* B3, double* results, double* zonal, hipStream_t st);
static int tem_epilogue(temx_plan* pl, double* results, double* zonal, hipStream_t st);
static int bin_project_op(temx_plan* pl, const void* A, int dtype, int64_t D, double* B, hipStream_t st);
static int bin_zonal_mean(temx_plan* pl, const void* A, int dtype, int64_t D, double* out, int native, hipStream_t st);
static int miss_check(const temx_plan* pl);
static int miss_zonal_mean(temx_plan* pl, const void* A, int dtype, int64_t D, double* out, int native, hipStream_t st);
static int tracer_stage3_impl(temx_plan* pl, const double* Bq2, double* tres, double* tzon, hipStream_t st);

static SliceMap slice_map(const temx_plan* pl, int nsl, int64_t rows_total, int64_t row0) {
  SliceMap m;
  if (nsl <= 1) return m;
  m.D = pl->D;
  m.nt = (int)pl->nt;
  m.W = nsl;
  m.chunk = rows_total * pl->nlev * ((pl->nt + nsl - 1) / nsl);
  m.row0 = row0;
  return m;
}

template <int NBK>
static int launch_osc_t(temx_plan* pl, const OscFieldsIn& fin, int nf, int nout, double* Bf, double* At, double* ab,
                        const OscPairsIn& pin, int np, double* Bp, int64_t Dt, hipStream_t st) {
  const unsigned gx = (unsigned)((Dt + 15) / 16);
  hipLaunchKernelGGL((osc_fields_kernel<NBK>), dim3(gx, nf, 2), dim3(OSC_W * 64), (size_t)osc_fields_lds(NBK) * 8, st, fin, pl->osc, pl->K,
                     pl->KX, pl->KR, pl->NQ, Dt, nout, Bf, At, ab, pl->D, (int)pl->tnt, (int)pl->nt, (int)pl->tt0);
  HIPCHK(hipGetLastError());
  hipLaunchKernelGGL((osc_pairs_kernel<NBK>), dim3(gx, np), dim3(OSC_W * 64), (size_t)osc_pairs_lds(NBK) * 8, st, pin, pl->osc, pl->wq2.d(),
                     pl->K, pl->KX, pl->NQ, Dt, Bp);
  HIPCHK(hipGetLastError());
  return TEMX_OK;
}
static int launch_osc(temx_plan* pl, const OscFieldsIn& fin, int nf, int nout, double* Bf, double* At, double* ab,
                      const OscPairsIn& pin, int np, double* Bp, int64_t Dt, hipStream_t st) {
  if (pl->TB == 13 && pl->TBX == 13) return launch_osc_t<13>(pl, fin, nf, nout, Bf, At, ab, pin, np, Bp, Dt, st);
  if (pl->TB == 8 && pl->TBX == 8) return launch_osc_t<8>(pl, fin, nf, nout, Bf, At, ab, pin, np, Bp, Dt, st);
  if (pl->TB == 4 && pl->TBX == 4) return launch_osc_t<4>(pl, fin, nf, nout, Bf, At, ab, pin, np, Bp, Dt, st);
  return fail(TEMX_EUNSUPPORTED, "single-sweep contraction: no instantiation for L = %d", pl->L);
}

static int os_prepass(temx_plan* pl, const FieldPtrs<4>& fp, int dtype, double* As, hipStream_t st) {
  int rc;
  const int64_t D = pl->D, KD4 = (int64_t)4 * pl->KX * D;
  pl->op_valid = pl->c4_valid = pl->tq_valid = pl->os_valid = false;
  if ((rc = launch_sweep_os<0>(pl, fp, dtype, true, pl->rho0.d(), pl->partial.d(), pl->sp_os_s, st))) return rc;
  return launch_reduce_rows(pl, pl->partial.d(), pl->sp_os_s.nsplit, KD4, 4, pl->KX, pl->KR, D, As, st);
}

static int os_sweep(temx_plan* pl, const FieldPtrs<4>& fp, int dtype, const double* As, int nsl, double* proj, hipStream_t st) {
  int rc;
  const int64_t D = pl->D;
  const int64_t KD4 = (int64_t)4 * pl->KX * D, KD3 = (int64_t)3 * pl->K * D;
  pl->op_valid = pl->c4_valid = pl->tq_valid = pl->os_valid = false;
  hipLaunchKernelGGL(os_ref_solve_kernel, dim3((unsigned)((D + 15) / 16), 4), dim3(256), 0, st, As, pl->KR, pl->KR, D,
                     pl->Gsinv.d(), pl->rho.d());
  HIPCHK(hipGetLastError());
  TimedLaunch tl{};
  time_begin(pl, 0, st, tl);
  rc = launch_sweep_os<0>(pl, fp, dtype, false, pl->rho.d(), pl->partial.d(), pl->sp_os, st);
  time_end(pl, 0, st, tl);
  if (rc) return rc;
  const int64_t rows = (int64_t)4 * pl->KX + 3 * pl->K;
  if ((rc = launch_reduce(pl, pl->partial.d(), pl->sp_os.nsplit, KD4, proj, st, -1, nullptr, slice_map(pl, nsl, rows, 0)))) return rc;
  return launch_reduce(pl, pl->partial.d() + (int64_t)pl->sp_os.nsplit * KD4, pl->sp_os.nsplit, KD3, nsl > 1 ? proj : proj + KD4, st, -1,
                       nullptr, slice_map(pl, nsl, rows, (int64_t)4 * pl->KX));
}

static int os_tail(temx_plan* pl, const double* proj_s, int64_t t0, int64_t nts, double* results, double* zonal, hipStream_t st) {
  int rc;
  set_tail(pl, t0, nts);
  const int64_t Dt = pl->tD;
  const int64_t rows = (int64_t)4 * pl->KX + 3 * pl->K;
  if (proj_s != pl->Ax.d())
    HIPCHK(hipMemcpyAsync(pl->Ax.p, proj_s, (size_t)rows * Dt * 8, hipMemcpyDeviceToDevice, st));
  {
    TimedLaunch t2{};
    time_begin(pl, 1, st, t2);
    const size_t lds = os_contract_lds(pl->K, pl->KX, pl->NQ) * 8;
    const double* Pp = pl->Ax.d() + (int64_t)4 * pl->KX * Dt;
    if (pl->osc_lds) {
      OsFields in;
      for (int f = 0; f < 4; ++f) {
        in.A[f] = pl->Ax.d() + (int64_t)f * pl->KX * Dt;
        in.rho[f] = pl->rho.d() + (int64_t)f * pl->KR * pl->D;
      }
      rc = launch_lds<os_contract_kernel<0>, 160 * 1024>(pl->device, dim3((unsigned)((Dt + OSC - 1) / OSC)), dim3(256), lds,
          st, in, Pp, pl->K, pl->KX, pl->KR, pl->NQ, Dt, pl->T.d(), pl->Ginv.d(), pl->G.d(), pl->Gx.d(), pl->gaunt.d(),
          pl->wq2.d(), pl->B4.d(), pl->B3.d(), pl->D, (int)nts, (int)pl->nt, (int)t0);
      if (rc) return rc;
    } else {
      using KD = OsKind<0>;
      const int64_t QD = (int64_t)pl->NQ * Dt;
      OscFieldsIn fin;
      OscPairsIn pin{};
      for (int f = 0; f < 4; ++f) {
        fin.A[f] = pl->Ax.d() + (int64_t)f * pl->KX * Dt;
        fin.rho[f] = pl->rho.d() + (int64_t)f * pl->KR * pl->D;
      }
      for (int k = 0; k < 3; ++k) {
        pin.At_a[k] = pl->osAt.d() + KD::pa(k) * QD; pin.At_b[k] = pl->osAt.d() + KD::pb(k) * QD;
        pin.ab_a[k] = pl->osAb.d() + KD::pa(k) * QD; pin.ab_b[k] = pl->osAb.d() + KD::pb(k) * QD;
        pin.P[k] = Pp + (int64_t)k * pl->K * Dt;
      }
      if ((rc = launch_osc(pl, fin, 4, 4, pl->B4.d(), pl->osAt.d(), pl->osAb.d(), pin, 3, pl->B3.d(), Dt, st))) return rc;
    }
    time_end(pl, 1, st, t2);
  }
  if ((rc = launch_solve(pl, pl->B4.d(), 4, Dt, pl->C4.d(), pl->zb.d(), st))) return rc;
  if ((rc = tem_stage3_impl(pl, pl->B3.d(), results, zonal, st))) return rc;
  pl->c4_valid = true;
  pl->os_valid = true;
  return TEMX_OK;
}

static int tem_run_os(temx_plan* pl, const FieldPtrs<4>& fp, int dtype, double* results, double* zonal, void* stream) {
  hipStream_t st = S_(stream);
  int rc;
  if ((rc = os_prepass(pl, fp, dtype, pl->Axs.d(), st))) return rc;
  if ((rc = os_sweep(pl, fp, dtype, pl->Axs.d(), 1, pl->Ax.d(), st))) return rc;
  return os_tail(pl, pl->Ax.d(), 0, pl->nt, results, zonal, st);
}

static int tracer_ws(temx_plan* pl);

static int tracer_os_ws(temx_plan* pl, int nq) {
  const int64_t D = pl->D;
  int rc;
  if ((rc = tracer_ws(pl))) return rc;
  if ((rc = pl->Axq.ensure((size_t)nq * (pl->KX + 2 * pl->K + pl->KR) * D * 8))) return rc;
  if ((rc = pl->osAtq.ensure((size_t)nq * pl->NQ * D * 8))) return rc;
  if ((rc = pl->osAbq.ensure((size_t)nq * pl->NQ * D * 8))) return rc;
  if ((rc = pl->Bqp.ensure((size_t)nq * 3 * pl->K * D * 8))) return rc;
  return pl->rho_t.ensure((size_t)4 * pl->KR * D * 8);
}

static int tracer_os_prepass(temx_plan* pl, int nq, const FieldPtrs<4>& fp, int dtype, double* Asq, hipStream_t st) {
  int rc;
  const int64_t D = pl->D;
  if ((rc = tracer_os_ws(pl, nq))) return rc;
  pl->tq_valid = false;
  rc = nq == 2 ? launch_sweep_os<3>(pl, fp, dtype, true, pl->rho0.d(), pl->partial.d(), pl->sp_os_s, st)
               : launch_sweep_os<1>(pl, fp, dtype, true, pl->rho0.d(), pl->partial.d(), pl->sp_os_s, st);
  if (rc) return rc;
  return launch_reduce_rows(pl, pl->partial.d(), pl->sp_os_s.nsplit, (int64_t)nq * pl->KX * D, nq, pl->KX, pl->KR, D, Asq, st);
}

static int tracer_os_sweep(temx_plan* pl, int nq, const FieldPtrs<4>& fp, int dtype, const double* Asq, int nsl, double* projq,
                           hipStream_t st) {
  int rc;
  const int64_t D = pl->D, KXD = (int64_t)pl->KX * D, KD = (int64_t)pl->K * D, KRD = (int64_t)pl->KR * D;
  if ((rc = tracer_os_ws(pl, nq))) return rc;
  pl->tq_valid = false;
  hipLaunchKernelGGL(os_ref_solve_kernel, dim3((unsigned)((D + 15) / 16), nq), dim3(256), 0, st, Asq, pl->KR, pl->KR, D,
                     pl->Gsinv.d(), pl->rho_t.d());
  HIPCHK(hipGetLastError());
  HIPCHK(hipMemcpyAsync(pl->rho_t.d() + nq * KRD, pl->rho.d() + 1 * KRD, (size_t)KRD * 8, hipMemcpyDeviceToDevice, st));
  HIPCHK(hipMemcpyAsync(pl->rho_t.d() + (nq + 1) * KRD, pl->rho.d() + 3 * KRD, (size_t)KRD * 8, hipMemcpyDeviceToDevice, st));
  rc = nq == 2 ? launch_sweep_os<3>(pl, fp, dtype, false, pl->rho_t.d(), pl->partial.d(), pl->sp_os, st)
               : launch_sweep_os<1>(pl, fp, dtype, false, pl->rho_t.d(), pl->partial.d(), pl->sp_os, st);
  if (rc) return rc;
  const int64_t rows = (int64_t)nq * (pl->KX + 2 * pl->K);
  if ((rc = launch_reduce(pl, pl->partial.d(), pl->sp_os.nsplit, nq * KXD, projq, st, -1, nullptr, slice_map(pl, nsl, rows, 0)))) return rc;
  return launch_reduce(pl, pl->partial.d() + (int64_t)pl->sp_os.nsplit * nq * KXD, pl->sp_os.nsplit, 2 * nq * KD,
                       nsl > 1 ? projq : projq + nq * KXD, st, -1, nullptr, slice_map(pl, nsl, rows, (int64_t)nq * pl->KX));
}

static int tracer_os_tail(temx_plan* pl, int nq, const double* projq_s, double* const* tres, double* const* tzon, hipStream_t st) {
  int rc;
  const int64_t Dt = pl->tD, KXD = (int64_t)pl->KX * Dt, KDt = (int64_t)pl->K * Dt, KRD = (int64_t)pl->KR * pl->D;
  double* Bq = pl->Bqp.d();
  double* Bq2 = pl->Bqp.d() + nq * KDt;
  if (pl->osc_lds) {
    if (nq != 1) return fail(TEMX_EUNSUPPORTED, "two tracers per sweep need the contraction on the matrix cores (TEMX_OPT_OS_CONTRACT = 0)");
    const size_t lds = os_contract_lds(pl->K, pl->KX, pl->NQ) * 8;
    OsFields in{};
    in.A[0] = projq_s;
    in.A[1] = pl->Ax.d() + 1 * KXD;
    in.A[2] = pl->Ax.d() + 3 * KXD;
    in.rho[0] = pl->rho_t.d();
    in.rho[1] = pl->rho.d() + 1 * KRD;
    in.rho[2] = pl->rho.d() + 3 * KRD;
    rc = launch_lds<os_contract_kernel<1>, 160 * 1024>(pl->device, dim3((unsigned)((Dt + OSC - 1) / OSC)), dim3(256), lds,
        st, in, projq_s + KXD, pl->K, pl->KX, pl->KR, pl->NQ, Dt, pl->T.d(), pl->Ginv.d(), pl->G.d(), pl->Gx.d(),
        pl->gaunt.d(), pl->wq2.d(), Bq, Bq2, pl->D, (int)pl->tnt, (int)pl->nt, (int)pl->tt0);
    if (rc) return rc;
  } else {
    const int64_t QD = (int64_t)pl->NQ * Dt;
    OscFieldsIn fin{};
    OscPairsIn pin{};
    const int other[2] = {1, 3};
    for (int i = 0; i < nq; ++i) {
      fin.A[i] = projq_s + i * KXD;
      fin.rho[i] = pl->rho_t.d() + i * KRD;
      for (int k = 0; k < 2; ++k) {
        const int p = 2 * i + k;
        pin.At_a[p] = pl->osAtq.d() + i * QD; pin.ab_a[p] = pl->osAbq.d() + i * QD;
        pin.At_b[p] = pl->osAt.d() + other[k] * QD; pin.ab_b[p] = pl->osAb.d() + other[k] * QD;
        pin.P[p] = projq_s + nq * KXD + (int64_t)p * KDt;
      }
    }
    if ((rc = launch_osc(pl, fin, nq, nq, Bq, pl->osAtq.d(), pl->osAbq.d(), pin, 2 * nq, Bq2, Dt, st))) return rc;
  }
// ... 1043 lines not shown
  if (int rc = upload(pl->Gx, Gx_host, (size_t)pl->K * pl->KX * 8)) return rc;
  pl->h_Gx.assign(Gx_host, Gx_host + (size_t)pl->K * pl->KX);
  if (int rc = os_upload_blocks(pl)) return rc;
  pl->os_need_global = false;
  pl->os_valid = false;
  return TEMX_OK;
} TEMX_CATCH

int temx_project(temx_plan* pl, const void* A, int dtype, int64_t D, double* B, void* stream) try {
  if (pl && miss_mode(pl)) return miss_refuse("temx_project");
  if (!pl || !A || !B) return fail(TEMX_EINVAL, "null argument");
  if (D < 1 || D >= ((int64_t)1 << 28)) return fail(TEMX_EINVAL, "D must be in [1, 2^28)");
  HIPCHK(hipSetDevice(pl->device));
  if (bin_mode(pl)) return bin_project_op(pl, A, dtype, D, B, S_(stream));
  FieldPtrs<1> fp;
  fp.p[0] = A;
  if (pl->cls) {
    Split spc = choose_split(D, std::max<int64_t>(1, pl->cbatches / 4), CLS_PROJ_E_WPS * pl->num_cu, 4);
    int rcc = pl->partial.ensure((size_t)spc.nsplit * pl->K * D * 8);
    if (rcc) return rcc;
    if ((rcc = launch_project_cls<1>(pl, fp, dtype, D, nullptr, -1, pl->partial.d(), spc, S_(stream)))) return rcc;
    return launch_reduce(pl, pl->partial.d(), spc.nsplit, (int64_t)pl->K * D, B, S_(stream));
  }
  Split sp = choose_split(D, pl->nchunk, 2 * pl->num_cu);
  int rc = pl->partial.ensure((size_t)sp.nsplit * std::min(pl->K, 64) * D * 8);
  if (rc) return rc;
  return project_all<1>(pl, fp, dtype, D, nullptr, -1, sp, B, S_(stream));
} TEMX_CATCH

int temx_zonal_mean_from_sums(temx_plan* pl, const double* B, int64_t D, double* out, int native,
                              void* stream) try {
  if (pl && miss_mode(pl)) return miss_refuse("temx_zonal_mean_from_sums");
  if (pl && bin_refused(pl)) return bin_refuse("temx_zonal_mean_from_sums");
  if (!pl || !B || !out) return fail(TEMX_EINVAL, "null argument");
  if (!pl->finalized) return fail(TEMX_ESTATE, "plan not finalised");
  HIPCHK(hipSetDevice(pl->device));
  int rc;
  if (!native) return launch_solve(pl, B, 1, D, nullptr, out, S_(stream));
  if ((rc = pl->opC.ensure((size_t)pl->K4 * D * 8))) return rc;
  if ((rc = launch_solve(pl, B, 1, D, pl->opC.d(), nullptr, S_(stream)))) return rc;
  return launch_recon(pl, D, pl->opC.d(), out, S_(stream));
} TEMX_CATCH

int temx_zonal_mean(temx_plan* pl, const void* A, int dtype, int64_t D, double* out, int native,
                    void* stream) try {
  if (!pl || !A || !out) return fail(TEMX_EINVAL, "null argument");
  if (!pl->finalized) return fail(TEMX_ESTATE, "plan not finalised");
  if (miss_mode(pl)) return miss_zonal_mean(pl, A, dtype, D, out, native, S_(stream));
  if (bin_mode(pl)) return bin_zonal_mean(pl, A, dtype, D, out, native, S_(stream));
  int rc = pl->opB.ensure((size_t)pl->K * std::max<int64_t>(D, 1) * 8);
  if (rc) return rc;
  if ((rc = temx_project(pl, A, dtype, D, pl->opB.d(), stream))) return rc;
  return temx_zonal_mean_from_sums(pl, pl->opB.d(), D, out, native, stream);
} TEMX_CATCH

struct FormChoice {
  bool two_pass;
  bool force_op;
  int os;
};
static FormChoice form_choice(const temx_plan* pl) {
  FormChoice c{false, false, -1};
  if (bin_mode(pl)) return FormChoice{true, false, 0};
  switch (pl->opt_form) {
    case TEMX_FORM_TWO_PASS: c.two_pass = true; c.os = 0; break;
    case TEMX_FORM_CLASS_SUMS: c.force_op = true; c.os = 0; break;
    case TEMX_FORM_SINGLE_SWEEP: c.force_op = true; c.os = 1; break;
    case TEMX_FORM_NO_SINGLE_SWEEP: c.os = 0; break;
    default: break;
  }
  if (const char* e = getenv("TEMX_TWO_PASS")) c.two_pass = e[0] == '1';
  if (const char* e = getenv("TEMX_ONE_PASS")) c.force_op = c.force_op || e[0] == '1';
  if (const char* e = getenv("TEMX_SINGLE_SWEEP")) c.os = e[0] == '0' ? 0 : (e[0] == '1' ? 1 : c.os);
  return c;
}
static bool tile_map(int opt, const char* env) {
  if (const char* e = getenv(env)) return !strcmp(e, "tile");
  return opt == 1;
}
static bool os_barrier_wanted(const temx_plan* pl) {
  if (const char* e = getenv("TEMX_OS_SYNC")) return !strcmp(e, "barrier");
  return pl->opt_os_sync == 1;
}
static bool tracer_one_pass_wanted(const temx_plan* pl) {
  if (const char* e = getenv("TEMX_TRACER_ONE_PASS")) return e[0] == '1';
  return pl->opt_tracer_one_pass == 1;
}

static int bin_check(const temx_plan* pl);
static int bin_set_tem(temx_plan* pl);

int temx_plan_configure(temx_plan* pl, int option, int value) try {
  if (!pl) return fail(TEMX_EINVAL, "null plan");
  switch (option) {
    case TEMX_OPT_FORM:
      if (value < -1 || value > TEMX_FORM_NO_SINGLE_SWEEP) return fail(TEMX_EINVAL, "TEMX_OPT_FORM: unknown form %d", value);
      pl->opt_form = value;
      break;
    case TEMX_OPT_OS_MAP: pl->opt_os_map = value; break;
    case TEMX_OPT_OP_MAP: pl->opt_op_map = value; break;
    case TEMX_OPT_TRACER_ONE_PASS: pl->opt_tracer_one_pass = value; break;
    case TEMX_OPT_OS_SUBSAMPLE:
      if (value < 4) return fail(TEMX_EINVAL, "TEMX_OPT_OS_SUBSAMPLE: at least 4 class-groups");
      if (pl->os_built && value != pl->os_keep) return fail(TEMX_ESTATE, "the single-sweep tables of this plan are built: set the subsample before temx_plan_set_tem");
      pl->os_keep = value;
      break;
    case TEMX_OPT_SINGLE_SWEEP_MIN_GROUPS: pl->opt_single_sweep_min_groups = value; break;
    case TEMX_OPT_OS_CONTRACT: pl->opt_os_contract = value; break;
    case TEMX_OPT_MISSING:
      if (value != 0 && value != 1) return fail(TEMX_EINVAL, "TEMX_OPT_MISSING: 0 (raise) or 1 (mask), got %d", value);
      if (value == 1) {
        if (bin_mode(pl)) return fail(TEMX_EUNSUPPORTED, "missing-value mode is not available while latitude bins are in effect (TEMX_OPT_LAT_BINS)");
        if (int rc = miss_check(pl)) return rc;
      }
      pl->opt_missing = value;
      pl->miss_valid = false;
      break;
    case TEMX_OPT_MIN_COVERAGE:
      if (value < 0 || value > 1000) return fail(TEMX_EINVAL, "TEMX_OPT_MIN_COVERAGE: per mille in 0..1000, got %d", value);
      pl->opt_min_cov = value;
      break;
    case TEMX_OPT_MISSING_WEIGHT:
      if (value < 4 || value > 14) return fail(TEMX_EINVAL, "TEMX_OPT_MISSING_WEIGHT: tau = 10^-value, value in 4..14, got %d", value);
      pl->opt_miss_w = value;
      break;
    case TEMX_OPT_OS_SYNC:
      if (value != 0 && value != 1) return fail(TEMX_EINVAL, "TEMX_OPT_OS_SYNC: 0 (flags) or 1 (barriers), got %d", value);
      pl->opt_os_sync = value;
      break;
    case TEMX_OPT_LAT_BINS: {
      const int B = value == -1 ? BIN_DEFAULT : value;
      if (B != 0) {
        if (!bin_count_ok(B)) return fail(TEMX_EINVAL, "TEMX_OPT_LAT_BINS: 0 (off), -1 (default, %d) or one of 128, 256, 512, 1024, 2048, got %d", BIN_DEFAULT, value);
        if (int rc = bin_check(pl)) return rc;
        if (bin_degree(pl->L, B) == 0)
          return fail(TEMX_EINVAL, "TEMX_OPT_LAT_BINS: (L, B) = (%d, %d): no Chebyshev degree up to %d keeps the basis rows to %.0e; use more bins",
                      pl->L, B, BIN_MAX_DEGREE, BIN_BOUND);
      }
      pl->opt_lat_bins = B;
      pl->bin_J = B ? bin_degree(pl->L, B) : 0;
      break;
    }
    case TEMX_OPT_BIN_DEGREE: return fail(TEMX_EINVAL, "TEMX_OPT_BIN_DEGREE is chosen by the library (read it with temx_plan_option)");
    default: return fail(TEMX_EINVAL, "unknown option %d", option);
  }
  pl->tem = false;
  return TEMX_OK;
} TEMX_CATCH

int temx_plan_option(const temx_plan* pl, int option) try {
  if (!pl) return -1;
  switch (option) {
    case TEMX_OPT_FORM:
      if (miss_mode(pl)) return TEMX_FORM_MASKED;
      if (bin_mode(pl)) return TEMX_FORM_BINNED;
      return pl->os_on ? TEMX_FORM_SINGLE_SWEEP : ((pl->cls && pl->onepass) || (pl->lcls && pl->lone) ? TEMX_FORM_CLASS_SUMS : TEMX_FORM_TWO_PASS);
    case TEMX_OPT_OS_MAP: return tile_map(pl->opt_os_map, "TEMX_OS_MAP") ? 1 : 0;
    case TEMX_OPT_OP_MAP: return tile_map(pl->opt_op_map, "TEMX_OP_MAP") ? 1 : 0;
    case TEMX_OPT_TRACER_ONE_PASS: return tracer_one_pass_wanted(pl) ? 1 : 0;
    case TEMX_OPT_OS_SUBSAMPLE: return pl->os_keep;
    case TEMX_OPT_SINGLE_SWEEP_MIN_GROUPS: return pl->opt_single_sweep_min_groups;
    case TEMX_OPT_OS_CONTRACT: return pl->osc_lds ? 1 : 0;
    case TEMX_OPT_MISSING: return pl->opt_missing;
    case TEMX_OPT_MIN_COVERAGE: return pl->opt_min_cov;
    case TEMX_OPT_MISSING_WEIGHT: return pl->opt_miss_w;
    case TEMX_OPT_OS_SYNC: return os_barrier_wanted(pl) ? 1 : 0;
    case TEMX_OPT_LAT_BINS: return pl->opt_lat_bins;
    case TEMX_OPT_BIN_DEGREE: return pl->bin_J;
    default: return -1;
  }
} TEMX_CATCH

int temx_plan_set_tem(temx_plan* pl, int nlev, int64_t nt, const double* p_pa_host, double p0) try {
  if (!pl || !p_pa_host) return fail(TEMX_EINVAL, "null argument");
  if (nlev < 2 || nt < 1) return fail(TEMX_EINVAL, "need nlev >= 2 and nt >= 1");
  if ((int64_t)nlev * nt >= ((int64_t)1 << 28)) return fail(TEMX_EINVAL, "nlev*nt must be < 2^28");
  if (pl->M < 2) return fail(TEMX_EINVAL, "need at least 2 zonal-mean latitudes");
  HIPCHK(hipSetDevice(pl->device));
  std::vector<double> p(p_pa_host, p_pa_host + nlev);
  for (int j = 1; j < nlev; ++j)
    if (!(p[j] > p[j - 1])) return fail(TEMX_EINVAL, "pressure must be strictly ascending (front end flips)");
  pl->tem = false;
  pl->onepass = pl->lone = pl->op_valid = pl->xb_valid = pl->tq_valid = false;
  pl->os_on = pl->os_valid = false;
  pl->miss_valid = pl->mt_valid = false;
  pl->os_tile = tile_map(pl->opt_os_map, "TEMX_OS_MAP");
  {
    const char* e = getenv("TEMX_OS_CONTRACT");
    pl->osc_lds = e ? !strcmp(e, "lds") : pl->opt_os_contract == 1;
  }
  pl->op_tile = tile_map(pl->opt_op_map, "TEMX_OP_MAP");
  pl->os_barrier = os_barrier_wanted(pl);
  pl->nlev = nlev;
  pl->nt = nt;
  pl->D = (int64_t)nlev * nt;
  pl->tD = pl->D;
  pl->tnt = nt;
  pl->tt0 = 0;
  pl->p0 = p0;
  const int M = pl->M;
  const int64_t D = pl->D;
  int rc;
  const TemTables tt = tem_tables(p, nt, p0, pl->lat_out_deg);
  if ((rc = upload(pl->p, p))) return rc;
  if ((rc = upload(pl->pg, tt.pg))) return rc;
  if ((rc = upload(pl->lg, tt.lg))) return rc;
  if ((rc = upload(pl->coslat, tt.coslat))) return rc;
  if ((rc = upload(pl->fcor, tt.fcor))) return rc;
  if ((rc = upload(pl->colscale, tt.colscale))) return rc;

  const int ndt_ = (int)((D + 15) / 16);
  const int pdpw = proj_dpw(4, ndt_);
  pl->sp_proj4 = choose_split(D, pl->nchunk, proj_wps(4, pdpw) * pl->num_cu, pdpw);
  const int edpw = pick_dpw(ndt_, 4);
  pl->sp_eddy = choose_split(D, pl->nchunk / (8 / edpw), pl->num_cu, edpw);
  const size_t need =
      (size_t)std::max(pl->sp_proj4.nsplit * 4, pl->sp_eddy.nsplit * (8 / edpw) * 3) * pl->K * D * 8;
  if ((rc = pl->partial.ensure(need))) return rc;
  if ((rc = pl->B4.ensure((size_t)4 * pl->K * D * 8))) return rc;
  if ((rc = pl->B3.ensure((size_t)3 * pl->K * D * 8))) return rc;
  if ((rc = pl->C4.ensure((size_t)4 * pl->K4 * D * 8))) return rc;
  if ((rc = pl->zb.ensure((size_t)8 * M * D * 8))) return rc;
  pl->sp_proj1 = choose_split(D, pl->nchunk, 2 * pl->num_cu);
  if (unfused_stage2(pl)) {
    const size_t need3 = (size_t)pl->sp_proj1.nsplit * 3 * 64 * D * 8;
    if ((rc = pl->partial.ensure(std::max(need3, pl->partial.bytes)))) return rc;
  }
  pl->lone = false;
  pl->xb_valid = false;
  pl->op_valid = false;
  if (pl->lcls) {
    const size_t need_cs = (size_t)pl->cgroups * ndt_ * 14 * 64 * 8, need_pb = (size_t)pl->cgroups * ndt_ * 3 * 128 * 8;
    size_t fr = 0, tot = 0;
    if (ndt_ >= 4 && !form_choice(pl).two_pass && hipMemGetInfo(&fr, &tot) == hipSuccess &&
        (pl->csum.bytes >= need_cs || need_cs + need_pb < fr / 2) && alloc_write_stream(pl->csum, need_cs) == TEMX_OK &&
        pl->pbuf.ensure(need_pb) == TEMX_OK) {
      HIPCHK(hipMemset(pl->csum.p, 0, pl->csum.bytes));
      HIPCHK(hipMemset(pl->pbuf.p, 0, pl->pbuf.bytes));
      const int64_t cunits = std::max<int64_t>(1, pl->cbatches / 4);
      pl->sp_cproj4 = choose_split(D, cunits, TEMX_CLS_OP_WPS * pl->num_cu, 4, 8);
      pl->sp_cflux = choose_split(D, std::max<int64_t>(1, pl->cgroups / (8 / edpw)), pl->num_cu, edpw, TEMX_CLS_MINCHUNK);
      pl->sp_lflux = choose_split(D, std::max<int64_t>(1, pl->cgroups / 8), pl->num_cu, 1, TEMX_CLS_MINCHUNK);
      const size_t need4 = (size_t)pl->sp_cflux.nsplit * 4 * 64 * D * 8;
      if ((rc = pl->partial.ensure(std::max(need4, pl->partial.bytes)))) return rc;
      if ((rc = pl->Bs.ensure((size_t)4 * 64 * D * 8))) return rc;
      const int2* cuts_unused = nullptr;
      if ((rc = class_cuts_dev(pl, pl->sp_cproj4.nsplit, &cuts_unused, true))) return rc;
      pl->lone = true;
    }
  }
  if (pl->cls) {
    const bool quad = pick_dpw(ndt_, 4) == 4;
    const int64_t cunits = std::max<int64_t>(1, pl->cbatches / 4);
    pl->sp_cproj4 = choose_split(D, cunits, (quad ? 2 : CLS_PROJ_E_WPS) * pl->num_cu, quad ? 4 : 1, TEMX_CLS_MINCHUNK);
    Split sp_op = choose_split(D, cunits, TEMX_CLS_OP_WPS * pl->num_cu, 4, 8);
    pl->sp_cproj1 = choose_split(D, cunits, CLS_PROJ_E_WPS * pl->num_cu, 4, TEMX_CLS_MINCHUNK);
    pl->sp_ceddy = choose_split(D, cunits / (8 / edpw), pl->num_cu, edpw, TEMX_CLS_MINCHUNK);
    const size_t need3 = (size_t)std::max({pl->sp_cproj4.nsplit * 4, pl->sp_ceddy.nsplit * (8 / edpw) * 3,
                                           pl->sp_cproj1.nsplit}) * pl->K * D * 8;
    if ((rc = pl->partial.ensure(std::max(need3, pl->partial.bytes)))) return rc;
    pl->onepass = false;
    pl->op_valid = false;
    {
      const FormChoice fc = form_choice(pl);
      const bool force = fc.force_op;
      const bool quad_op = ndt_ >= 4 && (force || (double)pl->N * (double)D >= 1.2e7);
      if (quad_op && !fc.two_pass) {
        const size_t need_cs = (size_t)pl->cgroups * ndt_ * 8 * 64 * 8;
        size_t fr = 0, tot = 0;
        bool have = pl->csum.bytes >= need_cs;
        if (!have && hipMemGetInfo(&fr, &tot) == hipSuccess && need_cs < fr / 2 && alloc_write_stream(pl->csum, need_cs) == TEMX_OK) {
          HIPCHK(hipMemset(pl->csum.p, 0, pl->csum.bytes));
          have = true;
        }
        if (have) {
// ... 1620 lines not shown
```

### pytemdiags_amd/engine.py

```python
from __future__ import annotations

import ctypes as C

import numpy as np
import torch

from . import _lib
from ._lib import check

_DT = {torch.float64: _lib.F64, torch.float32: _lib.F32}


def _ptr(t):
    return C.c_void_p(t.data_ptr())


def _dbl(a):
    a = np.ascontiguousarray(a, dtype=np.float64)
    return a, a.ctypes.data_as(C.POINTER(C.c_double))


def lat_bins_value(lat_bins):
    if lat_bins is None or lat_bins is False:
        return 0
    if lat_bins is True:
        return -1
    if isinstance(lat_bins, (int, np.integer)) and (int(lat_bins) == 0 or int(lat_bins) in _lib.LAT_BINS_ALLOWED):
        return int(lat_bins)
    raise ValueError("lat_bins must be True, 0 or one of %s, got %r" % (_lib.LAT_BINS_ALLOWED, lat_bins))


class Plan:

    def __init__(self, lat_deg, lat_out_deg, L, device=0, defer_finalize=False, symmetry=True, classes=True, qr=True,
                 form=None, fp32_fields=False, lat_bins=None):
        self._h = C.c_void_p()
        self.lib = _lib.load()
        if isinstance(device, torch.device):
            device = device.index or 0
        self.device_index = int(device)
        self.device = torch.device("cuda", self.device_index)
        lat, plat = _dbl(lat_deg)
        lat_out, plat_out = _dbl(lat_out_deg)
        self.N, self.M, self.L, self.K = int(lat.size), int(lat_out.size), int(L), int(L) + 1
        self.lat_out = lat_out
        self.nlev = self.nt = self.D = None
        self.form_requested = "auto"
        check(self.lib.temx_plan_create(C.byref(self._h), self.device_index, self.N, self.L, self.M,
                                        plat, plat_out, (_lib.DEFER_FINALIZE if defer_finalize else 0)
                                        | (0 if symmetry else _lib.NO_SYMMETRY)
                                        | (0 if classes else _lib.NO_CLASSES)
                                        | (0 if qr else _lib.NO_QR)
                                        | (_lib.LAT_TOL_F32 if fp32_fields else 0)))
        if form is not None:
            self.configure(form=form)
        if lat_bins is not None:
            self.configure(lat_bins=lat_bins)

    @property
    def paired(self):
        return bool(self.lib.temx_plan_is_paired(self._h))

    @property
    def sweep_mode(self):
        return int(self.lib.temx_plan_sweep_mode(self._h))

    @property
    def one_pass(self):
        return bool(self.lib.temx_plan_one_pass(self._h))

    @property
    def single_sweep(self):
        return bool(self.lib.temx_plan_single_sweep(self._h))

    @property
    def tracer_one_pass(self):
        return self.one_pass and self.option(_lib.OPT_TRACER_ONE_PASS) == 1

    def configure(self, form=None, os_map=None, op_map=None, os_subsample=None, tracer_one_pass=None,
                  single_sweep_min_groups=None, os_contract=None, missing=None, min_coverage=None,
                  missing_weight=None, os_sync=None, lat_bins=None):
        def put(opt, val):
            check(self.lib.temx_plan_configure(self._h, opt, int(val)))
        if missing is not None:
            if missing not in _lib.MISSING_MODES:
                raise ValueError("missing must be 'raise' or 'mask', got %r" % (missing,))
            put(_lib.OPT_MISSING, _lib.MISSING_MODES[missing])
        if min_coverage is not None:
            mc = float(min_coverage)
            if not 0.0 <= mc <= 1.0:
                raise ValueError("min_coverage must lie in [0, 1], got %r" % (min_coverage,))
            put(_lib.OPT_MIN_COVERAGE, int(round(mc * 1000)))
        if missing_weight is not None:
            e = -np.log10(float(missing_weight))
            if not (float(missing_weight) > 0 and abs(e - round(e)) < 1e-9 and 4 <= round(e) <= 14):
                raise ValueError("missing_weight must be 10^-n with n in 4..14, got %r" % (missing_weight,))
            put(_lib.OPT_MISSING_WEIGHT, int(round(e)))
        if form is not None:
            put(_lib.OPT_FORM, _lib.FORMS[form] if isinstance(form, str) else form)
            self.form_requested = form
        for opt, val in ((_lib.OPT_OS_MAP, os_map), (_lib.OPT_OP_MAP, op_map)):
            if val is not None:
                put(opt, {"row": 0, "tile": 1}[val] if isinstance(val, str) else val)
        if os_subsample is not None:
            put(_lib.OPT_OS_SUBSAMPLE, os_subsample)
        if tracer_one_pass is not None:
            put(_lib.OPT_TRACER_ONE_PASS, 1 if tracer_one_pass else 0)
        if single_sweep_min_groups is not None:
            put(_lib.OPT_SINGLE_SWEEP_MIN_GROUPS, single_sweep_min_groups)
        if os_contract is not None:
            put(_lib.OPT_OS_CONTRACT, {"mfma": 0, "lds": 1}[os_contract] if isinstance(os_contract, str) else os_contract)
        if lat_bins is not None:
            put(_lib.OPT_LAT_BINS, lat_bins_value(lat_bins))
        if os_sync is not None:
            put(_lib.OPT_OS_SYNC, {"flags": 0, "barrier": 1}[os_sync] if isinstance(os_sync, str) else os_sync)
        self.nlev = self.nt = self.D = None

    def option(self, opt):
        return int(self.lib.temx_plan_option(self._h, int(opt)))

    @property
    def lat_bins(self):
        return self.option(_lib.OPT_LAT_BINS)

    @property
    def bin_degree(self):
        return self.option(_lib.OPT_BIN_DEGREE)

    @property
    def sweep_form(self):
        return _lib.FORM_NAMES.get(self.option(_lib.OPT_FORM), "two-pass")

    @property
    def missing(self):
        return "mask" if self.option(_lib.OPT_MISSING) == 1 else "raise"

    def coverage(self):
        D = getattr(self, "_cov_D", None) or self.D or 1
        out = torch.empty((self.M, D), dtype=torch.float64, device=self.device)
        check(self.lib.temx_get_matrix(self._h, _lib.MAT_COVERAGE, _ptr(out), self._stream()))
        return out

    def close(self):
        if getattr(self, "_h", None) is not None and self._h.value:
            self.lib.temx_plan_destroy(self._h)
            self._h = C.c_void_p()

    def __del__(self):
        try:
            self.close()
        except Exception:
            pass

    def _stream(self):
        return C.c_void_p(torch.cuda.current_stream(self.device).cuda_stream)

    def _field(self, A, D=None):
        if not isinstance(A, torch.Tensor):
            raise TypeError("device tensors expected")
        if A.device != self.device:
            raise ValueError("tensor on %s, plan on %s" % (A.device, self.device))
        if A.dtype not in _DT:
            raise TypeError("dtype must be float64 or float32, got %s" % A.dtype)
        if A.shape[0] != self.N:
            raise ValueError("leading dimension must be ncol = %d" % self.N)
        A = A.contiguous()
        if D is not None and A.numel() != self.N * D:
            raise ValueError("field has %d elements, expected %d x %d" % (A.numel(), self.N, D))
        return A

    def finalize(self, G=None):
        if G is None:
            check(self.lib.temx_plan_finalize(self._h, None))
        else:
            g, pg = _dbl(G)
            assert g.shape == (self.K, self.K)
            check(self.lib.temx_plan_finalize(self._h, pg))

    def refine(self, G2=None):
        if G2 is None:
            check(self.lib.temx_plan_refine(self._h, None))
        else:
            g, pg = _dbl(G2)
            assert g.shape == (self.K, self.K)
            check(self.lib.temx_plan_refine(self._h, pg))

    def set_weights(self, weights):
        w, pw = _dbl(weights)
        assert w.size == self.N
        check(self.lib.temx_plan_set_weights(self._h, pw))

    def matrix(self, which):
        shape = {_lib.MAT_Y0: (self.N, self.K), _lib.MAT_Y0P: (self.M, self.K),
                 _lib.MAT_GRAM: (self.K, self.K), _lib.MAT_GINV: (self.K, self.K),
                 _lib.MAT_GRAM2: (self.K, self.K),
                 _lib.MAT_GX: (self.K, self.KX), _lib.MAT_GSUB: (self.KR, self.KR),
                 _lib.MAT_Y0INV: (self.K, self.N)}[which]
        out = torch.empty(shape, dtype=torch.float64, device=self.device)
# ... 589 lines not shown
```

Measured before the change: 186.7 billion grid-points/s.

## Add lean pre-pass sweep variant and merge reduce/solve chains in single-sweep path

Adds a PRE instantiation of the single-sweep kernel that computes only the projection sums needed by the reference pre-pass. It skips the eddy-product, rho-correction and LDS staging work, and allows two workgroups per CU. It also fuses the pre-pass partial reduction into the reference solve kernel, merges the two post-sweep reduce launches into one two-range reduce, and pairs the B4/B3 solves into one launch. These cut kernel launches and redundant memory passes, at the cost of more code paths and extra template variants. Each change can be switched off through new options.

```diff
diff --git a/include/temx.h b/include/temx.h
--- a/include/temx.h
+++ b/include/temx.h
@@ -43,7 +43,10 @@
   TEMX_OPT_MISSING_WEIGHT = 10,
   TEMX_OPT_LAT_BINS = 12,
   TEMX_OPT_BIN_DEGREE = 13,
-  TEMX_OPT_OS_SYNC = 11
+  TEMX_OPT_OS_SYNC = 11,
+  TEMX_OPT_OS_PREPASS = 14,
+  TEMX_OPT_OS_CHAIN = 15,
+  TEMX_OPT_OS_PREPASS_SPLITS = 16
 };
 enum {
   TEMX_FORM_AUTO = -1,
diff --git a/pytemdiags_amd/_lib.py b/pytemdiags_amd/_lib.py
--- a/pytemdiags_amd/_lib.py
+++ b/pytemdiags_amd/_lib.py
@@ -19,6 +19,9 @@
 OPT_MISSING, OPT_MIN_COVERAGE, OPT_MISSING_WEIGHT = 8, 9, 10
 OPT_OS_SYNC = 11
 OPT_LAT_BINS, OPT_BIN_DEGREE = 12, 13
+OPT_OS_PREPASS = 14
+OPT_OS_PREPASS_SPLITS = 16
+OPT_OS_CHAIN = 15
 LAT_BINS_ALLOWED = (128, 256, 512, 1024, 2048)
 LAT_BINS_DEFAULT = 512
 MISSING_MODES = {"raise": 0, "mask": 1}
diff --git a/pytemdiags_amd/csrc/kernels.hpp b/pytemdiags_amd/csrc/kernels.hpp
--- a/pytemdiags_amd/csrc/kernels.hpp
+++ b/pytemdiags_amd/csrc/kernels.hpp
@@ -269,6 +269,55 @@
   if (!(fabs(t) <= 1.79769313486231570815e308)) atomicOr(flag, 1);
 }
 
+__device__ __forceinline__ const double* two_range_src(const double* partial, int64_t stride1, int64_t n1,
+                                                       const double* partial2, int64_t stride2, int64_t idx,
+                                                       int64_t& stride) {
+  if (idx < n1) { stride = stride1; return partial + idx; }
+  stride = stride2;
+  return partial2 + (idx - n1);
+}
+__global__ void __launch_bounds__(256)
+reduce_partials2_kernel(const double* __restrict__ partial, int nsplit, int64_t stride1, int64_t n1,
+                        const double* __restrict__ partial2, int64_t stride2, int64_t n, double* __restrict__ B,
+                        int* __restrict__ flag) {
+  __shared__ double sh[16][17];
+  const int e = threadIdx.x & 15, sl = threadIdx.x >> 4;
+  const int64_t idx = (int64_t)blockIdx.x * 16 + e;
+  double s = 0.0;
+  if (idx < n) {
+    int64_t stride;
+    const double* src = two_range_src(partial, stride1, n1, partial2, stride2, idx, stride);
+    for (int sp = sl; sp < nsplit; sp += 16) s += src[(int64_t)sp * stride];
+  }
+  sh[sl][e] = s;
+  __syncthreads();
+  if (sl == 0 && idx < n) {
+    double t = 0.0;
+#pragma unroll
+    for (int j = 0; j < 16; ++j) t += sh[j][e];
+    B[idx] = t;
+    if (!(fabs(t) <= 1.79769313486231570815e308)) atomicOr(flag, 1);
+  }
+}
+template <int NS>
+__global__ void __launch_bounds__(256)
+reduce_partials_flat2_kernel(const double* __restrict__ partial, int nsplit, int64_t stride1, int64_t n1,
+                             const double* __restrict__ partial2, int64_t stride2, int64_t n, double* __restrict__ B,
+                             int* __restrict__ flag) {
+  const int64_t idx = (int64_t)blockIdx.x * 256 + threadIdx.x;
+  if (idx >= n) return;
+  int64_t stride;
+  const double* src = two_range_src(partial, stride1, n1, partial2, stride2, idx, stride);
+  double v[NS];
+#pragma unroll
+  for (int sp = 0; sp < NS; ++sp) v[sp] = src[(int64_t)(sp < nsplit ? sp : 0) * stride];
+  double t = 0.0;
+#pragma unroll
+  for (int sp = 0; sp < NS; ++sp) t += sp < nsplit ? v[sp] : 0.0;
+  B[idx] = t;
+  if (!(fabs(t) <= 1.79769313486231570815e308)) atomicOr(flag, 1);
+}
+
 __global__ void __launch_bounds__(256)
 reduce_rows_kernel(const double* __restrict__ partial, int nsplit, int64_t stride, int nf, int rows_in, int rows,
                    int64_t D, double* __restrict__ out, int* __restrict__ flag) {
@@ -367,24 +416,39 @@
   }
 }
 
+struct SolveSet2 {
+  const double* B2;
+  double* Xb2;
+  int nf1, mbs2;
+};
 constexpr int SOLVE_MB = 16;
 
-template <int TB>
+template <int TB, bool PAIR = false>
 __global__ void __launch_bounds__(256)
 solve_mfma_kernel(const double* __restrict__ B, int K, int M, int64_t D, const double* __restrict__ gblk,
                   const double* __restrict__ ypblk, double* __restrict__ C, double* __restrict__ Xb,
-                  int mbs ) {
+                  int mbs , SolveSet2 s2) {
   extern __shared__ double slds[];
   double* sg = slds;
   double* sy = slds + TB * TB * 16;
-  const int f = blockIdx.y;
+  int f = blockIdx.y;
+  const int nmb_all = (M + 3) >> 2;
+  if constexpr (PAIR) {
+    if (f >= s2.nf1) {
+      f -= s2.nf1;
+      B = s2.B2;
+      C = nullptr;
+      Xb = s2.Xb2;
+      mbs = s2.mbs2;
+    }
+    if ((int)blockIdx.z * mbs >= nmb_all) return;
+  }
   const int tid = threadIdx.x, lane = tid & 63, wave = tid >> 6;
   const int g = lane >> 4, c = lane & 15;
   const int64_t d = ((int64_t)blockIdx.x * 4 + wave) * 16 + c;
   const bool dvalid = d < D;
   const int64_t dcl = dvalid ? d : D - 1;
   const int mb0 = blockIdx.z * mbs;
-  const int nmb_all = (M + 3) >> 2;
   const int nmb = Xb != nullptr ? (nmb_all - mb0 < mbs ? nmb_all - mb0 : mbs) : 0;
 
   double breg[TB];
diff --git a/pytemdiags_amd/csrc/kernels_op2.hpp b/pytemdiags_amd/csrc/kernels_op2.hpp
--- a/pytemdiags_amd/csrc/kernels_op2.hpp
+++ b/pytemdiags_amd/csrc/kernels_op2.hpp
@@ -604,8 +604,8 @@
 __device__ __forceinline__ uint32_t handoff_look(const uint32_t* ctr) {
   return __hip_atomic_load(ctr, __ATOMIC_RELAXED, __HIP_MEMORY_SCOPE_WORKGROUP);
 }
-template <typename T, int TBS, int TBX, int NBR, int PD, int KIND = 0, int SYNC = 0>
-__global__ void __launch_bounds__(256, 1)
+template <typename T, int TBS, int TBX, int NBR, int PD, int KIND = 0, int SYNC = 0, int PRE = 0>
+__global__ void __launch_bounds__(256, PRE ? 2 : 1)
 sweep_osr_kernel(FieldPtrs<4> fp, int64_t D, int K, int KX, const double* __restrict__ ycx,
                  const int4* __restrict__ crow, const int2* __restrict__ csplit,
                  const double* __restrict__ colscale, const double* __restrict__ rho, int K4,
@@ -617,8 +617,11 @@
   constexpr int YJ = (YE + 255) / 256;
   constexpr int MB = CLS_MB;
   constexpr int NCH = 4;
-  constexpr int NV = 2 * (NF + NP);
+  constexpr int NV = PRE ? 2 * NF : 2 * (NF + NP);
   constexpr int NPR = KD::NPR, NPL = NP - NPR;
+  constexpr int NAX = PRE ? 2 * NBR : NBX;
+  constexpr int CBW = PRE ? 0 : NF * 2 * NBR * 64, APW = PRE ? 0 : NPL * 2 * TBS * 64;
+  static_assert(!PRE || (KIND == 0 && sizeof(T) == 8), "the pre-pass instantiation: TEM kind, fp64 fields");
   static_assert(NBR <= TBS && TBS <= TBX, "reference degree <= L <= 2L");
   static_assert(YJ <= 2, "Y quarter per thread");
   static_assert((PD - 1) * CLS_MB * KD::NF + (CLS_MB - 1) * KD::NF + 2 <= 63, "the ring is counted in vmcnt (6 bits)");
@@ -641,9 +644,9 @@
   const uint32_t aoff_r = (uint32_t)((lane & 3) * 4 + g);
   double* ybase = lds;
   double* cn = lds + 2 * YE;
-  double* cb = lds + 2 * YE + 16 + wave * (NF * 2 * NBR * 64) + lane;
-  double* apl = lds + 2 * YE + 16 + 4 * (NF * 2 * NBR * 64) + wave * (NPL * 2 * TBS * 64) + lane;
-  double* ex = lds + 2 * YE + 16 + 4 * (NF * 2 * NBR * 64) + 4 * (NPL * 2 * TBS * 64);
+  double* cb = lds + 2 * YE + 16 + wave * CBW + lane;
+  double* apl = lds + 2 * YE + 16 + 4 * CBW + wave * APW + lane;
+  double* ex = lds + 2 * YE + 16 + 4 * CBW + 4 * APW;
   double* exw = ex + wave * 64 + lane;
   const double* exr = ex + g * 64 + wave * 16 + c;
   uint32_t* hctr = reinterpret_cast<uint32_t*>(ex + NV * 256);
@@ -652,31 +655,35 @@
     if (tid < 2) hctr[tid] = 0u;
     __syncthreads();
   }
-#pragma unroll
-  for (int i = 0; i < NPL * 2 * TBS; ++i) apl[i * 64] = 0.0;
+  if constexpr (!PRE) {
+#pragma unroll
+    for (int i = 0; i < NPL * 2 * TBS; ++i) apl[i * 64] = 0.0;
+  }
   double apr[NPR > 0 ? NPR : 1][2 * TBS];
 #pragma unroll
   for (int k = 0; k < (NPR > 0 ? NPR : 1); ++k)
 #pragma unroll
     for (int t = 0; t < 2 * TBS; ++t) apr[k][t] = 0.0;
-#pragma unroll
-  for (int f = 0; f < NF; ++f)
-#pragma unroll
-    for (int tb = 0; tb < 2 * NBR; ++tb) {
-      const int l = tb < NBR ? 2 * (4 * tb + g) : 2 * (4 * (tb - NBR) + g) + 1;
-      const double v = rho[((int64_t)f * K4 + (l < K ? l : K - 1)) * D + dcl];
-      cb[(f * 2 * NBR + tb) * 64] = l < K ? v : 0.0;
-    }
+  if constexpr (!PRE) {
+#pragma unroll
+    for (int f = 0; f < NF; ++f)
+#pragma unroll
+      for (int tb = 0; tb < 2 * NBR; ++tb) {
+        const int l = tb < NBR ? 2 * (4 * tb + g) : 2 * (4 * (tb - NBR) + g) + 1;
+        const double v = rho[((int64_t)f * K4 + (l < K ? l : K - 1)) * D + dcl];
+        cb[(f * 2 * NBR + tb) * 64] = l < K ? v : 0.0;
+      }
+  }
   uint64_t fbase[NF];
 #pragma unroll
   for (int f = 0; f < NF; ++f) fbase[f] = reinterpret_cast<uint64_t>(fp.p[f]);
   { double sth_ready = sth; asm volatile("" : "+v"(sth_ready)); }
 
-  double ax[NFX][NBX];
+  double ax[NFX][NAX];
 #pragma unroll
   for (int f = 0; f < NFX; ++f)
 #pragma unroll
-    for (int t = 0; t < NBX; ++t) ax[f][t] = 0.0;
+    for (int t = 0; t < NAX; ++t) ax[f][t] = 0.0;
   double s[NF], q[NP], x0[NF], cnt = 0.0;
   double sN[NF], qN[NP], x0N[NF], cntN = 0.0;
 #pragma unroll
@@ -716,11 +723,13 @@
     constexpr int C = decltype(cc)::value;
 #pragma unroll
     for (int t = C * NBX / NCH; t < (C + 1) * NBX / NCH; ++t) {
+      const int tp = t < TBX ? t : t - TBX;
+      if (PRE && tp >= NBR) continue;
+      const int tx = PRE ? (t < TBX ? tp : NBR + tp) : t;
       const double ya = yprev[t * 16 + aoff_p];
 #pragma unroll
-      for (int f = 0; f < NFX; ++f) ax[f][t] = TEMX_MFMA4(ya, dS[f][t < TBX ? 0 : 1], ax[f][t]);
-      const int tp = t < TBX ? t : t - TBX;
-      if (tp < TBS) {
+      for (int f = 0; f < NFX; ++f) ax[f][tx] = TEMX_MFMA4(ya, dS[f][t < TBX ? 0 : 1], ax[f][tx]);
+      if (!PRE && tp < TBS) {
         const int ta = t < TBX ? tp : TBS + tp;
 #pragma unroll
         for (int k = 0; k < NPR; ++k) apr[k][ta] = TEMX_MFMA4(ya, dP[k][t < TBX ? 0 : 1], apr[k][ta]);
@@ -739,8 +748,10 @@
   auto park_north = [&]() __attribute__((always_inline)) {
 #pragma unroll
     for (int f = 0; f < NF; ++f) { sN[f] = s[f]; x0N[f] = x0[f]; s[f] = 0.0; }
-#pragma unroll
-    for (int k = 0; k < NP; ++k) { qN[k] = q[k]; q[k] = 0.0; }
+    if constexpr (!PRE) {
+#pragma unroll
+      for (int k = 0; k < NP; ++k) { qN[k] = q[k]; q[k] = 0.0; }
+    }
     cntN = cnt;
     cnt = 0.0;
   };
@@ -749,19 +760,19 @@
 #pragma unroll
     for (int f = 0; f < NF; ++f) {
       m2[0][f] = exr[f * 256];
-      m2[1][f] = exr[(NF + NP + f) * 256];
+      m2[1][f] = exr[(PRE ? NF + f : NF + NP + f) * 256];
     }
 #pragma unroll
     for (int k = 0; k < NP; ++k) {
-      c2[0][k] = exr[(NF + k) * 256];
-      c2[1][k] = exr[(2 * NF + NP + k) * 256];
+      c2[0][k] = PRE ? 0.0 : exr[(NF + k) * 256];
+      c2[1][k] = PRE ? 0.0 : exr[(2 * NF + NP + k) * 256];
     }
     const double nN = cn[g], nS = cn[4 + g];
     double E[NF], O[NF];
 #pragma unroll
     for (int f = 0; f < NF; ++f) E[f] = O[f] = 0.0;
 #pragma unroll
-    for (int tb = 0; tb < ((TEMX_OS_SKIP & 2) ? 0 : 2 * NBR); ++tb) {
+    for (int tb = 0; tb < (((TEMX_OS_SKIP & 2) || PRE) ? 0 : 2 * NBR); ++tb) {
       const int blk = tb < NBR ? tb : TBX + (tb - NBR);
       const double ya = yw[blk * 16 + aoff_r];
 #pragma unroll
@@ -776,10 +787,12 @@
       asm volatile("s_waitcnt lgkmcnt(0)" ::: "memory");
       if (lane == 0) __hip_atomic_fetch_add(&hctr[1], 1u, __ATOMIC_RELAXED, __HIP_MEMORY_SCOPE_WORKGROUP);
     }
-#pragma unroll
-    for (int f = 0; f < NF; ++f) {
-      m2[0][f] -= E[f] + O[f];
-      m2[1][f] -= E[f] - O[f];
+    if constexpr (!PRE) {
+#pragma unroll
+      for (int f = 0; f < NF; ++f) {
+        m2[0][f] -= E[f] + O[f];
+        m2[1][f] -= E[f] - O[f];
+      }
     }
 #pragma unroll
     for (int f = 0; f < NFX; ++f) {
@@ -787,12 +800,14 @@
       dS[f][0] = SNf + SSf;
       dS[f][1] = SNf - SSf;
     }
-#pragma unroll
-    for (int k = 0; k < NP; ++k) {
-      const double PNk = c2[0][k] + nN * m2[0][KD::pa(k)] * m2[0][KD::pb(k)];
-      const double PSk = c2[1][k] + nS * m2[1][KD::pa(k)] * m2[1][KD::pb(k)];
-      dP[k][0] = PNk + PSk;
-      dP[k][1] = PNk - PSk;
+    if constexpr (!PRE) {
+#pragma unroll
+      for (int k = 0; k < NP; ++k) {
+        const double PNk = c2[0][k] + nN * m2[0][KD::pa(k)] * m2[0][KD::pb(k)];
+        const double PSk = c2[1][k] + nS * m2[1][KD::pa(k)] * m2[1][KD::pb(k)];
+        dP[k][0] = PNk + PSk;
+        dP[k][1] = PNk - PSk;
+      }
     }
     yprev = yw;
     left = NCH;
@@ -866,8 +881,10 @@
       for (int f = 0; f < NF; ++f) dx[f] = (double)xb[P][j][f] - x0[f];
 #pragma unroll
       for (int f = 0; f < NF; ++f) s[f] += w * dx[f];
-#pragma unroll
-      for (int k = 0; k < NP; ++k) q[k] += (w * dx[KD::pa(k)]) * dx[KD::pb(k)];
+      if constexpr (!PRE) {
+#pragma unroll
+        for (int k = 0; k < NP; ++k) q[k] += (w * dx[KD::pa(k)]) * dx[KD::pb(k)];
+      }
       cnt += w;
     }
     if (fl & (CLS_LAST << 1)) {
@@ -889,13 +906,15 @@
       for (int f = 0; f < NF; ++f) {
         const double sc = f == KD::TF ? sth : 1.0;
         val[f] = (sN[f] * rnN + x0N[f]) * sc;
-        val[NF + NP + f] = (s[f] * rnS + x0[f]) * sc;
-      }
-#pragma unroll
-      for (int k = 0; k < NP; ++k) {
-        const double sc = k == KD::TP ? sth : 1.0;
-        val[NF + k] = (qN[k] - sN[KD::pa(k)] * sN[KD::pb(k)] * rnN) * sc;
-        val[2 * NF + NP + k] = (q[k] - s[KD::pa(k)] * s[KD::pb(k)] * rnS) * sc;
+        val[PRE ? NF + f : NF + NP + f] = (s[f] * rnS + x0[f]) * sc;
+      }
+      if constexpr (!PRE) {
+#pragma unroll
+        for (int k = 0; k < NP; ++k) {
+          const double sc = k == KD::TP ? sth : 1.0;
+          val[NF + k] = (qN[k] - sN[KD::pa(k)] * sN[KD::pb(k)] * rnN) * sc;
+          val[2 * NF + NP + k] = (q[k] - s[KD::pa(k)] * s[KD::pb(k)] * rnS) * sc;
+        }
       }
       if constexpr (SYNC == 0) {
         if (!(TEMX_OS_SKIP & 8)) asm volatile("s_waitcnt lgkmcnt(0)\n\ts_barrier" ::: "memory");
@@ -968,6 +987,18 @@
     static_for<NCH>([&](auto cc) __attribute__((always_inline)) {
       if (((decltype(cc)::value - first) & (NCH - 1)) < left) pending_chunk(cc);
     });
+  }
+  if constexpr (PRE) {
+    if (dvalid) {
+#pragma unroll
+      for (int f = 0; f < NFX; ++f)
+#pragma unroll
+        for (int t = 0; t < NAX; ++t) {
+          const int l = symx_harm<TBX>(t < NBR ? t : TBX + (t - NBR), g);
+          if (l < K4) px[(((int64_t)split * NFX + f) * KX + l) * D + d] = ax[f][t];
+        }
+    }
+    return;
   }
   if (dvalid) {
 #pragma unroll
@@ -1529,6 +1560,37 @@
   rho[((int64_t)f * KR + l) * D + d] = v0 + v1;
 }
 
+__global__ void __launch_bounds__(256)
+os_ref_solve_sum_kernel(const double* __restrict__ partial, int nsplit, int64_t stride, int rows_in, int KR, int64_t D,
+                        const double* __restrict__ Gsinv, double* __restrict__ As, double* __restrict__ rho,
+                        int* __restrict__ flag) {
+  __shared__ double sg[16 * 16];
+  __shared__ double sa[16 * 16];
+  const int f = blockIdx.y;
+  for (int i = threadIdx.x; i < KR * KR; i += blockDim.x) sg[i] = Gsinv[i];
+  const int dd = threadIdx.x & 15, l = threadIdx.x >> 4;
+  const int64_t d = blockIdx.x * (int64_t)16 + dd;
+  const bool ok = d < D && l < KR;
+  double t = 0.0;
+  if (ok) {
+    const double* src = partial + ((int64_t)f * rows_in + l) * D + d;
+    for (int sp = 0; sp < nsplit; ++sp) t += src[(int64_t)sp * stride];
+    As[((int64_t)f * KR + l) * D + d] = t;
+    if (!(fabs(t) <= 1.79769313486231570815e308)) atomicOr(flag, 1);
+  }
+  sa[l * 16 + dd] = t;
+  __syncthreads();
+  if (!ok) return;
+  double v0 = 0.0, v1 = 0.0;
+  int m = 0;
+  for (; m + 2 <= KR; m += 2) {
+    v0 += sg[l * KR + m] * sa[m * 16 + dd];
+    v1 += sg[l * KR + m + 1] * sa[(m + 1) * 16 + dd];
+  }
+  if (m < KR) v0 += sg[l * KR + m] * sa[m * 16 + dd];
+  rho[((int64_t)f * KR + l) * D + d] = v0 + v1;
+}
+
 constexpr int OSC = 4;
 constexpr int OSR = 256 / OSC;
 
diff --git a/pytemdiags_amd/csrc/temx.hip b/pytemdiags_amd/csrc/temx.hip
--- a/pytemdiags_amd/csrc/temx.hip
+++ b/pytemdiags_amd/csrc/temx.hip
@@ -167,6 +167,10 @@
   int opt_os_contract = -1;
   bool os_barrier = false;
   int opt_os_sync = -1;
+  bool os_prepass_full = false;
+  int opt_os_prepass = -1;
+  bool os_chain_sep = false;
+  int opt_os_chain = -1;
   int os_keep = 32;
   int64_t tD = 0, tnt = 0, tt0 = 0;
   int opt_form = -1, opt_os_map = -1, opt_op_map = -1, opt_tracer_one_pass = -1, opt_single_sweep_min_groups = -1;
@@ -408,6 +412,28 @@
   return TEMX_OK;
 }
 
+static int launch_reduce2(temx_plan* pl, const double* partial, int nsplit, int64_t n1, int64_t n2, double* B, hipStream_t st) {
+  const double* partial2 = partial + (int64_t)nsplit * n1;
+  const int64_t n = n1 + n2;
+  int* flag = static_cast<int*>(pl->flag.p);
+  if (nsplit <= 16 && std::max(n1, n2) >= 32768) {
+    const dim3 grid((unsigned)((n + 255) / 256));
+    if (nsplit <= 2)
+      hipLaunchKernelGGL(reduce_partials_flat2_kernel<2>, grid, dim3(256), 0, st, partial, nsplit, n1, n1, partial2, n2, n, B, flag);
+    else if (nsplit <= 4)
+      hipLaunchKernelGGL(reduce_partials_flat2_kernel<4>, grid, dim3(256), 0, st, partial, nsplit, n1, n1, partial2, n2, n, B, flag);
+    else if (nsplit <= 8)
+      hipLaunchKernelGGL(reduce_partials_flat2_kernel<8>, grid, dim3(256), 0, st, partial, nsplit, n1, n1, partial2, n2, n, B, flag);
+    else
+      hipLaunchKernelGGL(reduce_partials_flat2_kernel<16>, grid, dim3(256), 0, st, partial, nsplit, n1, n1, partial2, n2, n, B, flag);
+  } else {
+    hipLaunchKernelGGL(reduce_partials2_kernel, dim3((unsigned)((n + 15) / 16)), dim3(256), 0, st, partial, nsplit, n1, n1,
+                       partial2, n2, n, B, flag);
+  }
+  HIPCHK(hipGetLastError());
+  return TEMX_OK;
+}
+
 static int launch_reduce_rows(temx_plan* pl, const double* partial, int nsplit, int64_t stride, int nf, int rows_in,
                               int rows, int64_t D, double* out, hipStream_t st) {
   const int64_t n = (int64_t)nf * rows * D;
@@ -421,19 +447,26 @@
   return TEMX_OK;
 }
 
+static int solve_mbs(const temx_plan* pl, int NF, int64_t D) {
+  const int nmb = (pl->M + 3) / 4;
+  const int gx = (int)(((D + 15) / 16 + 3) / 4);
+  int mbs = SOLVE_MB;
+  while (mbs > 4 && (int64_t)gx * NF * ((nmb + mbs - 1) / mbs) < pl->num_cu / 2) mbs -= 4;
+  return mbs;
+}
+
 static int launch_solve(temx_plan* pl, const double* B, int NF, int64_t D, double* C, double* Xb,
                         hipStream_t st) {
   if (pl->K <= 64) {
     const int nmb = (pl->M + 3) / 4;
     const int gx = (int)(((D + 15) / 16 + 3) / 4);
-    int mbs = SOLVE_MB;
-    while (mbs > 4 && (int64_t)gx * NF * ((nmb + mbs - 1) / mbs) < pl->num_cu / 2) mbs -= 4;
+    const int mbs = solve_mbs(pl, NF, D);
     dim3 grid((unsigned)gx, NF, Xb ? (nmb + mbs - 1) / mbs : 1);
     return dispatch(TBValues{}, pl->TB, [&](auto tb) {
       constexpr int TBv = decltype(tb)::value;
       const size_t slds = ((size_t)TBv * TBv + (size_t)SOLVE_MB * TBv) * 16 * sizeof(double);
       return launch_lds<solve_mfma_kernel<TBv>>(pl->device, grid, dim3(256), slds, st, B, pl->K, pl->M, D, pl->gblk.d(),
-                                                pl->ypblk.d(), C, Xb, mbs);
+                                                pl->ypblk.d(), C, Xb, mbs, SolveSet2{});
     });
   }
   const int ms = Xb ? (pl->M + 63) / 64 : 1;
@@ -441,6 +474,23 @@
   const size_t slds = (size_t)2 * pl->K4 * 17 * sizeof(double);
   return launch_lds<solve_kernel, 160 * 1024>(pl->device, grid, dim3(1024), slds, st, B, pl->K, pl->K4, pl->M, D,
       pl->Ginv.d(), pl->Qp.d(), C, Xb);
+}
+
+static int launch_solve2(temx_plan* pl, const double* B1, int NF1, double* C1, double* Xb1, const double* B2, int NF2,
+                         double* Xb2, int64_t D, hipStream_t st) {
+  if (pl->K > 64 || !B1 || !B2 || !Xb1 || !Xb2 || NF1 < 1 || NF2 < 1)
+    return fail(TEMX_EINTERNAL, "launch_solve2: two right-hand-side sets with zonal means out, K <= 64");
+  const int nmb = (pl->M + 3) / 4;
+  const int gx = (int)(((D + 15) / 16 + 3) / 4);
+  const int mbs1 = solve_mbs(pl, NF1, D), mbs2 = solve_mbs(pl, NF2, D);
+  const int nz = std::max((nmb + mbs1 - 1) / mbs1, (nmb + mbs2 - 1) / mbs2);
+  dim3 grid((unsigned)gx, NF1 + NF2, nz);
+  return dispatch(TBValues{}, pl->TB, [&](auto tb) {
+    constexpr int TBv = decltype(tb)::value;
+    const size_t slds = ((size_t)TBv * TBv + (size_t)SOLVE_MB * TBv) * 16 * sizeof(double);
+    return launch_lds<solve_mfma_kernel<TBv, true>>(pl->device, grid, dim3(256), slds, st, B1, pl->K, pl->M, D,
+                                                    pl->gblk.d(), pl->ypblk.d(), C1, Xb1, mbs1, SolveSet2{B2, Xb2, NF1, mbs2});
+  });
 }
 
 template <typename T, int MODE, int KIND>
@@ -908,6 +958,19 @@
     constexpr size_t lds = ((size_t)2 * 2 * TBXv * 16 + 16 + (size_t)4 * KD::NF * 2 * NBR * 64 +
                             (size_t)4 * (KD::NP - KD::NPR) * 2 * TBSv * 64 + (size_t)2 * (KD::NF + KD::NP) * 256 + 2) * 8;
     static_assert(lds <= 163840, "the single sweep's workgroup fits the LDS of a compute unit");
+    if constexpr (KIND == 0) {
+      if (sub && !pl->os_prepass_full) {
+        constexpr size_t lds_pre = ((size_t)2 * 2 * TBXv * 16 + 16 + (size_t)2 * KD::NF * 256 + 2) * 8;
+        static_assert(2 * lds_pre <= 163840, "two pre-pass workgroups fit the LDS of a compute unit");
+        auto go_pre = [&](auto handoff) {
+          return launch_lds<sweep_osr_kernel<double, TBSv, TBXv, NBR, 2, 0, decltype(handoff)::value, 1>>(pl->device, grid,
+              block, lds_pre, st, fp, pl->D, pl->K, pl->KX, pl->ycx_s.d(), static_cast<const int4*>(pl->crow_s.p), cuts,
+              pl->colscale.d(), static_cast<const double*>(nullptr), pl->KR, px, static_cast<double*>(nullptr), sp.nsplit,
+              sp.ndt, static_cast<int*>(pl->flag.p) + 1);
+        };
+        return pl->os_barrier ? go_pre(Int<0>{}) : go_pre(Int<1>{});
+      }
+    }
     auto go = [&](auto handoff) {
       return launch_lds<sweep_osr_kernel<double, TBSv, TBXv, NBR, 2, KIND, decltype(handoff)::value>>(pl->device, grid,
           block, lds, st, fp, pl->D, pl->K, pl->KX, sub ? pl->ycx_s.d() : pl->ycx.d(),
@@ -989,16 +1052,24 @@
   const int64_t D = pl->D, KD4 = (int64_t)4 * pl->KX * D;
   pl->op_valid = pl->c4_valid = pl->tq_valid = pl->os_valid = false;
   if ((rc = launch_sweep_os<0>(pl, fp, dtype, true, pl->rho0.d(), pl->partial.d(), pl->sp_os_s, st))) return rc;
+  if (As == nullptr) return TEMX_OK;
   return launch_reduce_rows(pl, pl->partial.d(), pl->sp_os_s.nsplit, KD4, 4, pl->KX, pl->KR, D, As, st);
 }
-
-static int os_sweep(temx_plan* pl, const FieldPtrs<4>& fp, int dtype, const double* As, int nsl, double* proj, hipStream_t st) {
+static bool os_solve_sums(const temx_plan* pl) { return !pl->os_chain_sep && pl->sp_os_s.nsplit <= 16; }
+
+static int os_sweep(temx_plan* pl, const FieldPtrs<4>& fp, int dtype, const double* As, int nsl, double* proj, hipStream_t st,
+                    double* As_slabs = nullptr) {
   int rc;
   const int64_t D = pl->D;
   const int64_t KD4 = (int64_t)4 * pl->KX * D, KD3 = (int64_t)3 * pl->K * D;
   pl->op_valid = pl->c4_valid = pl->tq_valid = pl->os_valid = false;
-  hipLaunchKernelGGL(os_ref_solve_kernel, dim3((unsigned)((D + 15) / 16), 4), dim3(256), 0, st, As, pl->KR, pl->KR, D,
-                     pl->Gsinv.d(), pl->rho.d());
+  if (As_slabs != nullptr)
+    hipLaunchKernelGGL(os_ref_solve_sum_kernel, dim3((unsigned)((D + 15) / 16), 4), dim3(256), 0, st, pl->partial.d(),
+                       pl->sp_os_s.nsplit, KD4, pl->KX, pl->KR, D, pl->Gsinv.d(), As_slabs, pl->rho.d(),
+                       static_cast<int*>(pl->flag.p));
+  else
+    hipLaunchKernelGGL(os_ref_solve_kernel, dim3((unsigned)((D + 15) / 16), 4), dim3(256), 0, st, As, pl->KR, pl->KR, D,
+                       pl->Gsinv.d(), pl->rho.d());
   HIPCHK(hipGetLastError());
   TimedLaunch tl{};
   time_begin(pl, 0, st, tl);
@@ -1006,6 +1077,8 @@
   time_end(pl, 0, st, tl);
   if (rc) return rc;
   const int64_t rows = (int64_t)4 * pl->KX + 3 * pl->K;
+  if (nsl <= 1 && !pl->os_chain_sep)
+    return launch_reduce2(pl, pl->partial.d(), pl->sp_os.nsplit, KD4, KD3, proj, st);
   if ((rc = launch_reduce(pl, pl->partial.d(), pl->sp_os.nsplit, KD4, proj, st, -1, nullptr, slice_map(pl, nsl, rows, 0)))) return rc;
   return launch_reduce(pl, pl->partial.d() + (int64_t)pl->sp_os.nsplit * KD4, pl->sp_os.nsplit, KD3, nsl > 1 ? proj : proj + KD4, st, -1,
                        nullptr, slice_map(pl, nsl, rows, (int64_t)4 * pl->KX));
@@ -1051,8 +1124,13 @@
     }
     time_end(pl, 1, st, t2);
   }
-  if ((rc = launch_solve(pl, pl->B4.d(), 4, Dt, pl->C4.d(), pl->zb.d(), st))) return rc;
-  if ((rc = tem_stage3_impl(pl, pl->B3.d(), results, zonal, st))) return rc;
+  if (!pl->os_chain_sep && pl->K <= 64) {
+    if ((rc = launch_solve2(pl, pl->B4.d(), 4, pl->C4.d(), pl->zb.d(), pl->B3.d(), 3, pl->zb.d() + 4 * (int64_t)pl->M * Dt, Dt, st))) return rc;
+    if ((rc = tem_epilogue(pl, results, zonal, st))) return rc;
+  } else {
+    if ((rc = launch_solve(pl, pl->B4.d(), 4, Dt, pl->C4.d(), pl->zb.d(), st))) return rc;
+    if ((rc = tem_stage3_impl(pl, pl->B3.d(), results, zonal, st))) return rc;
+  }
   pl->c4_valid = true;
   pl->os_valid = true;
   return TEMX_OK;
@@ -1061,8 +1139,9 @@
 static int tem_run_os(temx_plan* pl, const FieldPtrs<4>& fp, int dtype, double* results, double* zonal, void* stream) {
   hipStream_t st = S_(stream);
   int rc;
-  if ((rc = os_prepass(pl, fp, dtype, pl->Axs.d(), st))) return rc;
-  if ((rc = os_sweep(pl, fp, dtype, pl->Axs.d(), 1, pl->Ax.d(), st))) return rc;
+  const bool sums = os_solve_sums(pl);
+  if ((rc = os_prepass(pl, fp, dtype, sums ? nullptr : pl->Axs.d(), st))) return rc;
+  if ((rc = os_sweep(pl, fp, dtype, pl->Axs.d(), 1, pl->Ax.d(), st, sums ? pl->Axs.d() : nullptr))) return rc;
   return os_tail(pl, pl->Ax.d(), 0, pl->nt, results, zonal, st);
 }
 
@@ -2272,6 +2351,14 @@
   if (const char* e = getenv("TEMX_OS_SYNC")) return !strcmp(e, "barrier");
   return pl->opt_os_sync == 1;
 }
+static bool os_prepass_full_wanted(const temx_plan* pl) {
+  if (const char* e = getenv("TEMX_OS_PREPASS")) return !strcmp(e, "full");
+  return pl->opt_os_prepass == 1;
+}
+static bool os_chain_sep_wanted(const temx_plan* pl) {
+  if (const char* e = getenv("TEMX_OS_CHAIN")) return !strcmp(e, "separate");
+  return pl->opt_os_chain == 1;
+}
 static bool tracer_one_pass_wanted(const temx_plan* pl) {
   if (const char* e = getenv("TEMX_TRACER_ONE_PASS")) return e[0] == '1';
   return pl->opt_tracer_one_pass == 1;
@@ -2318,6 +2405,14 @@
       if (value != 0 && value != 1) return fail(TEMX_EINVAL, "TEMX_OPT_OS_SYNC: 0 (flags) or 1 (barriers), got %d", value);
       pl->opt_os_sync = value;
       break;
+    case TEMX_OPT_OS_PREPASS:
+      if (value != 0 && value != 1) return fail(TEMX_EINVAL, "TEMX_OPT_OS_PREPASS: 0 (lean) or 1 (full), got %d", value);
+      pl->opt_os_prepass = value;
+      break;
+    case TEMX_OPT_OS_CHAIN:
+      if (value != 0 && value != 1) return fail(TEMX_EINVAL, "TEMX_OPT_OS_CHAIN: 0 (merged) or 1 (separate), got %d", value);
+      pl->opt_os_chain = value;
+      break;
     case TEMX_OPT_LAT_BINS: {
       const int B = value == -1 ? BIN_DEFAULT : value;
       if (B != 0) {
@@ -2332,6 +2427,7 @@
       break;
     }
     case TEMX_OPT_BIN_DEGREE: return fail(TEMX_EINVAL, "TEMX_OPT_BIN_DEGREE is chosen by the library (read it with temx_plan_option)");
+    case TEMX_OPT_OS_PREPASS_SPLITS: return fail(TEMX_EINVAL, "TEMX_OPT_OS_PREPASS_SPLITS is chosen by the library (read it with temx_plan_option)");
     default: return fail(TEMX_EINVAL, "unknown option %d", option);
   }
   pl->tem = false;
@@ -2355,6 +2451,9 @@
     case TEMX_OPT_MIN_COVERAGE: return pl->opt_min_cov;
     case TEMX_OPT_MISSING_WEIGHT: return pl->opt_miss_w;
     case TEMX_OPT_OS_SYNC: return os_barrier_wanted(pl) ? 1 : 0;
+    case TEMX_OPT_OS_PREPASS: return os_prepass_full_wanted(pl) ? 1 : 0;
+    case TEMX_OPT_OS_CHAIN: return os_chain_sep_wanted(pl) ? 1 : 0;
+    case TEMX_OPT_OS_PREPASS_SPLITS: return pl->os_on ? pl->sp_os_s.nsplit : 0;
     case TEMX_OPT_LAT_BINS: return pl->opt_lat_bins;
     case TEMX_OPT_BIN_DEGREE: return pl->bin_J;
     default: return -1;
@@ -2381,6 +2480,8 @@
   }
   pl->op_tile = tile_map(pl->opt_op_map, "TEMX_OP_MAP");
   pl->os_barrier = os_barrier_wanted(pl);
+  pl->os_prepass_full = os_prepass_full_wanted(pl);
+  pl->os_chain_sep = os_chain_sep_wanted(pl);
   pl->nlev = nlev;
   pl->nt = nt;
   pl->D = (int64_t)nlev * nt;
diff --git a/pytemdiags_amd/engine.py b/pytemdiags_amd/engine.py
--- a/pytemdiags_amd/engine.py
+++ b/pytemdiags_amd/engine.py
@@ -79,7 +79,7 @@
 
     def configure(self, form=None, os_map=None, op_map=None, os_subsample=None, tracer_one_pass=None,
                   single_sweep_min_groups=None, os_contract=None, missing=None, min_coverage=None,
-                  missing_weight=None, os_sync=None, lat_bins=None):
+                  missing_weight=None, os_sync=None, lat_bins=None, os_prepass=None, os_chain=None):
         def put(opt, val):
             check(self.lib.temx_plan_configure(self._h, opt, int(val)))
         if missing is not None:
@@ -114,6 +114,10 @@
             put(_lib.OPT_LAT_BINS, lat_bins_value(lat_bins))
         if os_sync is not None:
             put(_lib.OPT_OS_SYNC, {"flags": 0, "barrier": 1}[os_sync] if isinstance(os_sync, str) else os_sync)
+        if os_prepass is not None:
+            put(_lib.OPT_OS_PREPASS, {"lean": 0, "full": 1}[os_prepass] if isinstance(os_prepass, str) else os_prepass)
+        if os_chain is not None:
+            put(_lib.OPT_OS_CHAIN, {"merged": 0, "separate": 1}[os_chain] if isinstance(os_chain, str) else os_chain)
         self.nlev = self.nt = self.D = None
 
     def option(self, opt):
```

After: 187.2 billion grid-points/s, median of 2. Within noise of the previous version (+0.3%).
